# robin-karlsson0/pc-accumulation-lib

Measured on AMD Instinct MI355X. Metric: Mpoints/s projected+accumulated and BEV frames/s @256x256; 1/2/4/8 GPU, higher is better.
Workload: dtype f64; 1 GPU; KITTI-360 single forward cam, 120k pts/frame, 200 m horizon (~201 live frames, 5169634 stored pts), one 256x256x21 BEV per integrated frame; points_per_frame=120000, bev_px=256, view_m=80

## Files before the change

### include/pca.h

```cpp
#ifndef PCA_H
#define PCA_H

#include <stdint.h>

#ifdef __cplusplus
extern "C" {
#endif

#define PCA_VERSION 2

typedef struct pca_ctx pca_ctx;

typedef struct {
    double *x, *y, *z;
    float *intensity;
    uint32_t *rgbs;
    int32_t *inst;
    uint8_t *dyn;
    int64_t capacity;
    uint32_t *frame_box;
} pca_store;

#define PCA_STATUS_STORE_OVERFLOW 1u
#define PCA_STATUS_UV_OUT_OF_IMAGE 2u
#define PCA_STATUS_NEGATIVE_INTENSITY 4u
#define PCA_STATUS_LOOKBACK_TIMEOUT 8u
#define PCA_STATUS_LANES_BISECT_CAP 16u

int pca_version(void);
int pca_ctx_create(int device, pca_ctx **out);
void pca_ctx_destroy(pca_ctx *ctx);
const char *pca_last_error(pca_ctx *ctx);
int pca_status(pca_ctx *ctx, void *stream, uint32_t *status_out);
int pca_status_peek(pca_ctx *ctx, uint32_t *status_out);
const uint32_t *pca_status_mirror(pca_ctx *ctx);

typedef struct {
    const float *pts;
    const uint8_t *rgb;
    const uint8_t *sem;
    const uint8_t *sem_gt;
    int32_t n;
    int32_t reserved;
} pca_kitti_frame;

int pca_kitti_project_sample_filter(pca_ctx *ctx, const pca_kitti_frame *frames, int n_frames, const double P[12],
                                    int H, int W, const uint64_t filter_mask[4], const pca_store *store,
                                    int64_t *frame_off , int first_slot, void *stream);

#define PCA_SAMPLE_NEAREST 0
#define PCA_SAMPLE_BILINEAR 1
int pca_kitti_project_sample_filter_ex(pca_ctx *ctx, const pca_kitti_frame *frames, int n_frames, const double P[12],
                                       int H, int W, const uint64_t filter_mask[4], const pca_store *store,
                                       int64_t *frame_off , int first_slot, int sample_mode, void *stream);

int pca_nusc_sample_filter_transform(pca_ctx *ctx, const double *pc, const int64_t *cam_idx, int32_t n,
                                     const uint8_t *imgs, const uint8_t *sems, int ncam, int H, int W,
                                     const double T[16], const uint64_t filter_mask[4], const pca_store *store,
                                     int64_t *frame_off , int slot, void *stream);
int pca_nusc_sample_filter_transform_ex(pca_ctx *ctx, const double *pc, const int64_t *cam_idx, int32_t n,
                                        const uint8_t *imgs, const uint8_t *sems, int ncam, int H, int W,
                                        const double T[16], const uint64_t filter_mask[4], const pca_store *store,
                                        int64_t *frame_off , int slot, int sample_mode, void *stream);

typedef struct {
    const double *pc;
    const int64_t *cam_idx;
    const uint8_t *imgs;
    const uint8_t *sems;
    int32_t n;
    int32_t reserved;
    const double *T;
} pca_nusc_frame;
int pca_nusc_sample_filter_transform_batch(pca_ctx *ctx, const pca_nusc_frame *frames, int n_frames, int ncam, int H, int W,
                                           const uint64_t filter_mask[4], const pca_store *store, int64_t *frame_off ,
                                           int first_slot, int sample_mode, void *stream);

int pca_sample_bilinear(pca_ctx *ctx, const double *map , int H, int W, const double *uv , int32_t n,
                        double *out , void *stream);

int pca_nusc_project_cams(pca_ctx *ctx, const double *pc_lidar, int32_t n, const double T_ego_from_lidar[16],
                          const double T_glob_from_ego[16], const double *T_cam_from_glob, const double *K,
                          const double *wh, int ncam, double *pc_in_ego, double *uv, int64_t *cam_idx,
                          void *stream);

#define PCA_NUSC_MAX_SWEEPS 32
#define PCA_NUSC_MAX_SWEEP_BOXES 4096
#define PCA_NUSC_MAX_SWEEP_TILES 16384
typedef struct {
    int32_t row0, n_rows;
    int32_t box0, n_boxes;
    float lag, sweep;
    double T[12];
} pca_nusc_sweep;
typedef struct {
    double inv[12];
    double size[3];
    int32_t cls;
    int32_t track_key;
} pca_nusc_sweep_box;
int64_t pca_nusc_merge_sweeps_workspace_bytes(int64_t n_points, int n_boxes);
int pca_nusc_merge_sweeps(pca_ctx *ctx, const float *raw , int64_t n_points, const pca_nusc_sweep *sweeps,
                          int n_sweeps, const pca_nusc_sweep_box *boxes, int n_boxes, float center_radius,
                          double inside_limit, void *workspace , int64_t workspace_bytes,
                          float *points_out , int32_t *tally_out , void *stream);

int pca_retransform(pca_ctx *ctx, const pca_store *store, const int64_t *frame_off , int slot_begin,
                    int slot_end, const double *Ts, int n_T, void *stream);

int pca_retransform_batch_tail(pca_ctx *ctx, const pca_store *store, const int64_t *frame_off , int first_slot,
                               int n_frames, const double *Ts, void *stream);

int pca_mark_dynamic(pca_ctx *ctx, const pca_store *store, const int64_t *frame_off , const int32_t *slots,
                     const int32_t *inst_idx, int n_pairs, void *stream);

int64_t pca_voxel_dedup_workspace_bytes(int64_t max_points, int n_slots);
int pca_voxel_dedup(pca_ctx *ctx, const pca_store *store, int64_t *frame_off , int slot_begin, int slot_end,
                    double voxel_size, int64_t max_points, void *workspace , int64_t workspace_bytes,
                    void *stream);

int64_t pca_icp_workspace_bytes(int32_t max_points);
int pca_icp_register(pca_ctx *ctx, const float *src_pts , int32_t n_src, const float *tgt_pts ,
                     int32_t n_tgt, double max_corr_dist, const double init[16], int max_iter, double rel_fitness,
                     double rel_rmse, void *workspace , int64_t workspace_bytes, double T_out[16],
                     double *fitness, double *rmse, int *iterations, void *stream);

typedef struct {
    double origin[3];
    double R[9];
    double dx, dy;
    double view;
    double height_filter;
    double int_scaler, int_sep_scaler, int_mid_threshold;
    double rgb_fill;
    int32_t px;
    int32_t road_class;
    uint64_t dynobj_mask[4];
    int32_t intensity_div255;
    int32_t pad;
} pca_bev_params;

int64_t pca_bev_workspace_bytes(int64_t max_points, int px);

int pca_bev_generate(pca_ctx *ctx, const pca_store *store, const double *intensity64,
                     const int64_t *frame_off , int slot_begin, int slot_split, int slot_end,
                     int64_t max_points, const pca_bev_params *prm, const double *pending_T, int pending_slot_end,
                     void *workspace , int64_t workspace_bytes, double *planes ,
                     uint16_t *planes_f16 , void *stream);

#define PCA_BEV_EXTRA_PLANES 3
int pca_bev_generate_ex(pca_ctx *ctx, const pca_store *store, const double *intensity64,
                        const int64_t *frame_off , int slot_begin, int slot_split, int slot_end,
                        int64_t max_points, const pca_bev_params *prm, const double *pending_T, int pending_slot_end,
                        void *workspace , int64_t workspace_bytes, double *planes ,
                        uint16_t *planes_f16 , double *extra_planes , void *stream);

#define PCA_BEV_MAX_CHAIN 4
int pca_bev_generate_chain(pca_ctx *ctx, const pca_store *store, const double *intensity64,
                           const int64_t *frame_off , int slot_begin, int slot_split, int slot_end,
                           int64_t max_points, const pca_bev_params *prm, const double *pending_Ts,
                           const int *pending_slot_ends, int n_pending, int write_back, void *workspace ,
                           int64_t workspace_bytes, double *planes , uint16_t *planes_f16 ,
                           double *extra_planes , void *stream);

typedef struct {
    int32_t slot_begin, slot_split, slot_end, reserved;
    pca_bev_params prm;
    double *planes;
    uint16_t *planes_f16;
} pca_bev_job;
int pca_bev_generate_many(pca_ctx *ctx, const pca_store *store, const double *intensity64 ,
                          const int64_t *frame_off , const pca_bev_job *jobs, int n_jobs, int64_t max_points,
                          void *workspace , int64_t workspace_bytes, void *stream);

#define PCA_BEV_MAX_CLASS_GROUPS 16
typedef struct { uint64_t mask[4]; } pca_class_group;
int64_t pca_bev_class_workspace_bytes(int64_t max_points, int px);
int pca_bev_class_planes(pca_ctx *ctx, const pca_store *store, const int64_t *frame_off ,
                         int slot_begin, int slot_split, int slot_end, int64_t max_points,
                         const pca_bev_params *prm,
                         const pca_class_group *groups, int n_groups,
                         const double *pending_Ts, const int *pending_slot_ends, int n_pending,
                         void *workspace , int64_t workspace_bytes,
                         double *prob      ,
                         uint16_t *prob_f16,
                         uint32_t *counts  ,
                         void *stream);

int64_t pca_bev_elev_workspace_bytes(int64_t max_points, int px);
int pca_bev_elev_partition(pca_ctx *ctx, const pca_store *store, const int64_t *frame_off ,
                           int slot_begin, int slot_end, int64_t max_points,
                           const pca_bev_params *prm, double elev_thresh, int include_dyn,
                           const double *pending_Ts, const int *pending_slot_ends, int n_pending,
                           void *workspace , int64_t workspace_bytes,
                           double *elev      ,
                           uint8_t *observed ,
                           uint8_t *flags    ,
                           int64_t *counts   ,
                           void *stream);

int pca_image_to_nchw_f32(pca_ctx *ctx, const uint8_t *rgb , int H, int W, const float mean[3], const float std[3],
                          float *out , void *stream);

int pca_bev_warp(pca_ctx *ctx, const uint16_t *planes_f16 , uint16_t *out_f16 , int n_planes, int px,
                 double a_1, double a_2, double b_1, double b_2, void *stream);

int pca_host_ego_to_grid(const double *full, int F, const double R[9], double dx, double dy, double view, int px,
                         double *rows, int32_t *start);

typedef struct {
    double origin[3];
    double R[9];
    double dx, dy, view;
    int32_t px, reserved;
} pca_lane_view;
int64_t pca_lanes_workspace_bytes(int64_t n_vertices, int n_samples, int64_t cap_rows);
int pca_lanes_transform(pca_ctx *ctx, double *xyz , int64_t P, const double T[16], void *stream);
int pca_lanes_to_grid(pca_ctx *ctx, const double *xyz , const int32_t *vertex_lane , const int32_t *start ,
                      int64_t P, int32_t L, const pca_lane_view *views , int S, int64_t cap_rows,
                      double *rows , int32_t *row_lane , int64_t *n_rows , void *ws,
                      void *stream);

typedef struct pca_host_track pca_host_track;
typedef struct {
    const void *pts;
    const void *rgb;
    const void *sem;
    const void *sem_gt;
    int32_t n;
    uint32_t host_mask;
} pca_kitti_obs;
int pca_kitti_integrate(pca_ctx *ctx, const pca_kitti_obs *obs, const double P[12], int H, int W,
                        const uint64_t filter_mask[4], const pca_store *store, int64_t *frame_off , int slot,
                        int sample_mode, pca_host_track *track, const double *T_new_prev, double horizon, int64_t *evicted,
                        double *path_length, void *stream);
void pca_host_camera_cone(const double P[12], int H, int W, double cone[15]);
int pca_host_view_hull(int F, const double *then , const float *box , const double *cone ,
                       const double now[12], const pca_bev_params *prm, int *first, int *last);
int pca_bev_bin_range(pca_ctx *ctx, int slot_first, int slot_last_plus1);
int pca_bev_view_hint(pca_ctx *ctx, int slot0, int F, const double *then, const float *box, const double *cone, const double now[12],
                      const pca_bev_params *prm);
void pca_f32_box_decode(const uint32_t *rows , int n, float *box );

int pca_debug_bev_level1(const pca_ctx *ctx, int out[4]);
int pca_debug_icp_layout(int32_t n_src, int32_t n_tgt, int64_t out[16]);

int pca_k1_defer(pca_ctx *ctx, int on);
int pca_k1_flush(pca_ctx *ctx);
int pca_kitti_generate_bev(pca_ctx *ctx, const pca_store *store, const int64_t *frame_off , int slot_begin,
                           int slot_split, int slot_end, int64_t max_points, const pca_bev_params *prm,
                           const double *pending_Ts, const int *pending_slot_ends, int n_pending, int write_back,
                           void *workspace , int64_t workspace_bytes, uint16_t *planes_f16 ,
                           void *host_planes , const pca_host_track *track, double *traj_rows,
                           int32_t *traj_start, int32_t *n_rows, void *stream);

typedef struct {
    const pca_kitti_obs *obs; const double *P; int32_t H, W; const uint64_t *filter_mask; const pca_store *store;
    int64_t *frame_off; int32_t slot, sample_mode; pca_host_track *track; const double *T_new_prev; double horizon;
    int64_t evicted; double path_length; void *stream;
} pca_kitti_integrate_args;
int pca_kitti_integrate_v(pca_ctx *ctx, pca_kitti_integrate_args *a);
typedef struct {
    const pca_store *store; const int64_t *frame_off; int32_t slot_begin, slot_split, slot_end, pad0; int64_t max_points;
    const pca_bev_params *prm; const double *pending_Ts; const int *pending_slot_ends; int32_t n_pending, write_back;
    void *workspace; int64_t workspace_bytes; uint16_t *planes_f16; void *host_planes; const pca_host_track *track;
    double *traj_rows; int32_t *traj_start; int32_t n_rows, pad1; void *stream;
    int32_t hint_slot0, hint_F; const double *hint_then; const float *hint_box; const double *hint_cone; const double *hint_now;
    int32_t hinted, pad2;
} pca_kitti_generate_bev_args;
int pca_kitti_generate_bev_v(pca_ctx *ctx, pca_kitti_generate_bev_args *a);

int pca_host_stage_h2d(int n, const void *const *src, void *const *pinned, void *const *dev, const int64_t *bytes,
                       void *stream);

int pca_host_d2h_async(pca_ctx *ctx, const void *dev, void *pinned, int64_t bytes, void *stream);
int pca_host_d2h_wait(pca_ctx *ctx, int ticket);

#define PCA_DEFLATE_CHUNK_MAX 32768
#define PCA_DEFLATE_MAX_CHUNKS (1 << 20)
#define PCA_DEFLATE_BOUND(n) ((9 * (int64_t)(n) + 7) / 8 + 16)
typedef struct { int64_t offset; int32_t length; int32_t reserved; } pca_deflate_chunk;
int64_t pca_deflate_workspace_bytes(int64_t n_chunks);
int pca_deflate_chunks(pca_ctx *ctx, const void *src , const pca_deflate_chunk *chunk_table , int64_t n_chunks,
                       void *out , uint32_t *out_sizes , uint32_t *out_crcs , void *workspace ,
                       void *stream);
int pca_deflate_chunks_dyn(pca_ctx *ctx, const void *src , const pca_deflate_chunk *chunk_table , int64_t n_chunks,
                           void *out , uint32_t *out_sizes , uint32_t *out_crcs , void *workspace ,
                           void *stream);
uint32_t pca_host_crc32_combine(uint32_t crc_a, uint32_t crc_b, int64_t len_b);
int64_t pca_host_gzip_assemble(int32_t n_pieces, const void *const *piece, const int64_t *piece_bytes, const int64_t *raw_bytes,
                               const uint32_t *crc, void *out, int64_t out_cap);

typedef struct pca_host_track pca_host_track;
int pca_host_gemv4_probe(void *cblas_dgemv64, int mode, const double *T , const double *x , int64_t n,
                         double *y );
int pca_host_gemv4_mode(int mode);
int pca_host_incr_probe(void *cblas_dgemv64, const double *d, int64_t n, int64_t r0, int64_t r1, double *out);
int pca_host_incr_blocks(int on);
int pca_host_track_create(pca_host_track **out, void *cblas_dgemv64);
void pca_host_track_destroy(pca_host_track *t);
int64_t pca_host_track_len(const pca_host_track *t);
int64_t pca_host_track_n_segments(const pca_host_track *t);
const double *pca_host_track_poses(const pca_host_track *t);
const double *pca_host_track_segments(const pca_host_track *t);
int pca_host_track_set(pca_host_track *t, const double *poses , int64_t n, const double *segs, int64_t nd);
int pca_host_track_transform(pca_host_track *t, const double T[16]);
int pca_host_track_append(pca_host_track *t, const double pose[3]);
int pca_host_track_push_segment(pca_host_track *t, double *path_length);
int pca_host_track_incr(pca_host_track *t, double *out);
int64_t pca_host_track_evict_beyond(pca_host_track *t, double horizon, double path_length);
int64_t pca_host_track_step(pca_host_track *t, const double T_new_prev[16], double horizon, double *path_length);
int64_t pca_host_track_trigger(pca_host_track *t, double bev_horizon, int64_t previous_idx, double min_step);

enum {
    PCA_K_KITTI = 0, PCA_K_NUSC, PCA_K_PROJECT_CAMS, PCA_K_RETRANSFORM, PCA_K_MARK_DYNAMIC,
    PCA_K_BEV_BIN, PCA_K_BEV_SCAN, PCA_K_BEV_SCATTER, PCA_K_BEV_CELLS, PCA_K_BEV_CELLS_HEAVY, PCA_K_DEDUP, PCA_K_BEV_UNIT, PCA_K_ICP,
    PCA_K_BEV_CLASS_BIN, PCA_K_BEV_CLASS_CELLS, PCA_K_BEV_ELEV_BIN, PCA_K_BEV_ELEV_CELLS, PCA_K_COUNT
};
int pca_profile_enable(pca_ctx *ctx, int on);
int pca_profile_read(pca_ctx *ctx, int kernel_id, double *total_ms, int64_t *launches);

#ifdef __cplusplus
}
#endif
#endif
```

### pc-accumulation-lib_amd/bev_generator/bev_generator.py

```python
import os
import time
from abc import ABC, abstractmethod

import ctypes

import numpy as np

from pca_amd import host_logic as hl

SETS = ('present', 'future', 'full')
PLANES = ('road', 'intensity', 'r', 'g', 'b', 'dynamic', 'elevation')


class DeviceWindow:

    def __init__(self, store, split, origin, first=0, last=None, future_is_present=False):
        self.store = store
        self.split = int(split)
        self.origin = np.asarray(origin, dtype=np.float64)
        self.first = int(first)
        self.last = store.n_frames if last is None else int(last)
        self.future_is_present = bool(future_is_present)

    def part(self, name):
        return WindowPart(self, name)


class WindowPart:

    def __init__(self, window, name):
        self.window = window
        self.name = name

    def to_numpy(self):
        w = self.window
        rows = w.store.frame_rows()
        lo, hi = {'present': (w.first, w.split), 'future': (w.split, w.last), 'full': (w.first, w.last)}[self.name]
        if w.future_is_present:
            lo, hi = w.first, w.last
        out = np.concatenate(rows[lo:hi]) if hi > lo else np.zeros((0, 10))
        out[:, :3] = out[:, :3] - w.origin
        return out


class BEVGenerator(ABC):

    def __init__(self,
                 view_size: int,
                 pixel_size: int,
                 max_trans_radius: float = 0.,
                 zoom_thresh: float = 0.,
                 do_warp: bool = False,
                 int_scaler: float = 1.,
                 int_sep_scaler: float = 1.,
                 int_mid_threshold: float = 0.5,
                 height_filter=None):
        self.view_size = view_size
        self.pixel_size = pixel_size
        self.max_trans_radius = max_trans_radius
        self.zoom_thresh = zoom_thresh
        self.do_warp = do_warp
        self.do_aug = bool(self.max_trans_radius > 0. or self.zoom_thresh > 0.)
        self.int_scaler = int_scaler
        self.int_sep_scaler = int_sep_scaler
        self.int_mid_threshold = int_mid_threshold
        self.sem_idx = 7
        self.height_filter = height_filter
        if self.height_filter is not None:
            print("NOTE: Removes points above ego-vehicle height!")
        self._tmp = {}
        self._frame = None
        self._device_only = False
        self._out16 = None
        self._defer = None
        self._lane_defer = None

    def __getstate__(self):
        d = dict(self.__dict__)
        d['_tmp'] = {}
        d['_defer'] = None
        d['_lane_defer'] = None
        return d

    class _RasterBatch:
        def __init__(self, gen):
            self.gen = gen

        def __enter__(self):
            self.gen._defer = []
            return self

        def __exit__(self, exc_type, exc, tb):
            jobs, self.gen._defer = self.gen._defer, None
            if self.gen._lane_defer is not None:
                lane_jobs, self.gen._lane_defer = self.gen._lane_defer, None
                if exc_type is not None:
                    return False
                lanes = lane_jobs[0][0]
                assert all(j[0] is lanes for j in lane_jobs)
                lanes.to_grid([j[1] for j in lane_jobs], asynchronous=True, into=[j[2] for j in lane_jobs])
            if exc_type is None and jobs:
                store = jobs[0][0]
                assert all(j[0] is store for j in jobs)
                outs = [j[2] for j in jobs]
                base = outs[0]._base if outs[0]._base is not None else outs[0]
                px = int(jobs[0][1][1].px)
                contiguous = all(o.data_ptr() == base.data_ptr() + k * 21 * px * px * 2 for k, o in enumerate(outs))
                if len(jobs) > 1 and contiguous and base.numel() >= len(jobs) * 21 * px * px:
                    store.bev_many([j[1] for j in jobs], base.view(-1)[:len(jobs) * 21 * px * px].view(len(jobs), 21, px, px))
                else:
                    for _, (split, prm, first, last), out in jobs:
                        store.bev(split, prm, first_frame=first, last_frame=last, out16=out)
            return False

    def raster_batch(self):
        return BEVGenerator._RasterBatch(self)

    def _raster_params(self, origin, rot_mat, dx, dy, aug_view_size, intensity_div255):
        key = ('prm', bool(intensity_div255), self.pixel_size, self.height_filter, self.int_scaler,
               self.int_sep_scaler, self.int_mid_threshold, getattr(self, 'rgb_fill', 0))
        prm = self._tmp.get(key)
        if prm is None:
            from pca_amd.device_store import make_bev_params
            sem_idxs = getattr(self, 'sem_idxs', None) or {}
            dyn_cls = [sem_idxs[k] for k in ('car', 'truck', 'bus', 'motorcycle') if k in sem_idxs]
            prm = self._tmp[key] = make_bev_params(np.zeros(3), np.eye(3), 0., 0., 1., self.pixel_size,
                                                   self.height_filter, self.int_scaler, self.int_sep_scaler,
                                                   self.int_mid_threshold, sem_idxs.get('road', -1), dyn_cls,
                                                   intensity_div255, getattr(self, 'rgb_fill', 0))
        head = self._tmp.get(id(prm))
        if head is None:
            head = self._tmp[id(prm)] = np.frombuffer((ctypes.c_double * 15).from_address(ctypes.addressof(prm)), dtype=np.float64)
        head[0:3] = origin
        head[3:12] = np.asarray(rot_mat, dtype=np.float64).reshape(9)
        head[12], head[13], head[14] = dx, dy, aug_view_size
        return prm

    def _tmp_store(self, key):
        from pca_amd.device_store import DeviceStore
        if key not in self._tmp:
            self._tmp[key] = DeviceStore(capacity=1 << 16, max_frames=4)
        return self._tmp[key]

    def rasterise(self, pc_present, pc_future, pc_full, rot_mat, dx, dy, aug_view_size, want_f64=False, out16=None):
        if isinstance(pc_present, WindowPart):
            w = pc_present.window
            prm = self._raster_params(w.origin, rot_mat, dx, dy, aug_view_size, w.store.intensity_div255)
            if self._defer is not None and out16 is not None and not want_f64 and not w.future_is_present:
                from pca_amd._lib import PcaBevParams
                self._defer.append((w.store, (w.split, PcaBevParams.from_buffer_copy(prm), w.first, w.last), out16))
                return out16, None
            return w.store.bev(w.split, prm, want_f64=want_f64, first_frame=w.first, last_frame=w.last, out16=out16)
        zero = np.zeros(3)
        prm = self._raster_params(zero, rot_mat, dx, dy, aug_view_size, False)
        st = self._tmp_store('pf')
        i64 = st.load_rows([pc_present, pc_future])
        a16, a64 = st.bev(1, prm, want_f64=want_f64, intensity64=i64)
        st2 = self._tmp_store('full')
        i64 = st2.load_rows([pc_full])
        b16, b64 = st2.bev(1, prm, want_f64=want_f64, intensity64=i64)
        a16[14:21] = b16[0:7]
        if want_f64:
            a64[14:21] = b64[0:7]
        return a16, a64

    @abstractmethod
    def generate_bev(self, pc_present, pc_future, pc_full, trajs_present, trajs_future, trajs_full,
                     gt_lane_trajs=None):
        pass

    def generate(self,
                 pcs: dict,
                 trajs: dict,
                 rot_ang: float = 0.,
                 trans_dx: float = 0.,
                 trans_dy: float = 0.,
                 zoom_scalar: float = 1.,
                 do_warping: bool = False,
                 device_only: bool = False,
                 out=None):
        pc_present, pc_future, pc_full = self.extract_pc_dict(pcs)
        ego_present, ego_future, ego_full = self.extract_ego_traj_dict(trajs)
        oth_present, oth_future, oth_full = self.extract_other_traj_dicts(trajs)
        lanes = self.extract_gt_lane_dicts(trajs) if 'gt_lanes' in trajs.keys() else None

        aug_view_size = zoom_scalar * self.view_size
        if do_warping is False:
            rot_ang = hl.heading_rot_ang(ego_present)
        rot_mat = hl.rotation_matrix_3d(rot_ang)

        def to_grid(traj_list):
            return [hl.transform_traj(t, rot_mat, trans_dx, trans_dy, aug_view_size, self.pixel_size, mutate=False)
                    for t in traj_list]

        split = trajs.get('_ego_split')
        if split is not None and pc_future is not None:
            ego_p, ego_f, ego_a = hl.transform_ego_split(ego_full, split, rot_mat, trans_dx, trans_dy, aug_view_size,
                                                        self.pixel_size)
            trajs_present = [ego_p] + to_grid(oth_present)
            trajs_future = [ego_f] + to_grid(oth_future)
            trajs_full = [ego_a] + to_grid(oth_full)
        else:
            trajs_present = to_grid([ego_present] + oth_present)
        if lanes is not None and not isinstance(lanes, list):
            from pca_amd.lanes import LaneView, PendingLanes
            view = LaneView(lanes.origin, rot_mat, trans_dx, trans_dy, aug_view_size, self.pixel_size)
            if self._defer is not None and device_only:
                if self._lane_defer is None:
                    self._lane_defer = []
                pending = PendingLanes()
                self._lane_defer.append((lanes.lanes, view, pending))
                lanes = pending
            else:
                lanes = lanes.lanes.to_grid([view], asynchronous=device_only)[0]
                if not device_only:
                    lanes = lanes.resolve()
        elif lanes is not None:
            lanes = [lane for lane in to_grid(lanes) if lane.shape[0] > 0]
        if pc_future is None:
            raise UnboundLocalError("local variable 'trajs_future' referenced before assignment")
        if split is None:
            trajs_future = to_grid([ego_future] + oth_future)
            trajs_full = to_grid([ego_full] + oth_full)

        self._frame = (rot_mat, trans_dx, trans_dy, aug_view_size)
        self._device_only = device_only
        self._out16 = out if device_only else None
        return self.generate_bev(pc_present, pc_future, pc_full, trajs_present, trajs_future, trajs_full, lanes)

    def preprocess_pc_and_trajs(self, pc, trajs, rot_ang, trans_dx, trans_dy, aug_view_size):
        rot_mat = hl.rotation_matrix_3d(rot_ang)
        pc = self.geometric_transform(pc, rot_ang, trans_dx, trans_dy, aug_view_size)
        out_trajs = [hl.transform_traj(t, rot_mat, trans_dx, trans_dy, aug_view_size, self.pixel_size)
                     for t in trajs]
        if self.height_filter is not None:
            pc = pc[pc[:, 2] < self.height_filter]
        return self.pos2grid(pc, aug_view_size), out_trajs

    def generate_rand_aug(self, pcs: dict, trajs: dict, do_warping: bool = True, device_only: bool = False, out=None,
                          worker: int = 0):
        np.random.seed(((os.getpid() + int(worker)) * int(time.time())) % 123456789)
        rot_ang = 2 * np.pi * np.random.random()
        trans_r = self.max_trans_radius * np.random.random()
        trans_ang = 2 * np.pi * np.random.random()
        trans_dx = trans_r * np.cos(trans_ang)
        trans_dy = trans_r * np.sin(trans_ang)
        zoom_scalar = np.random.normal(0, 0.1)
        zoom_scalar = 1 + min(max(zoom_scalar, -self.zoom_thresh), self.zoom_thresh)
        return self.generate(pcs, trajs, rot_ang, trans_dx, trans_dy, zoom_scalar, do_warping, device_only, out)

    def generate_multiproc(self, bev_gen_inputs, device_only: bool = False, out=None, worker: int = 0):
        pcs, trajs = bev_gen_inputs
        if self.do_aug:
            return self.generate_rand_aug(pcs, trajs, device_only=device_only, out=out, worker=worker)
        return self.generate(pcs, trajs, device_only=device_only, out=out)

    def generate_rand_aug_multiproc(self, bev_gen_inputs):
        pcs, trajs = bev_gen_inputs
        return self.generate_rand_aug(pcs, trajs, do_warping=True)

    def geometric_transform(self, pc_mat, rot_ang, trans_dx, trans_dy, aug_view_size, is_traj=False):
        rot_mat = self.rotation_matrix_3d(rot_ang)
        pc_mat[:, :3] = np.matmul(rot_mat, pc_mat[:, :3].T).T
        pc_mat[:, 0] += trans_dx
        pc_mat[:, 1] += trans_dy
        if is_traj:
            return self.crop_trajectory(pc_mat, aug_view_size)
        return self.crop_view(pc_mat, aug_view_size)

    @staticmethod
    def crop_view(pc_mat, aug_view_size):
        h = 0.5 * aug_view_size
        pc_mat = pc_mat[np.logical_and(pc_mat[:, 0] > -h, pc_mat[:, 0] < h)]
        return pc_mat[np.logical_and(pc_mat[:, 1] > -h, pc_mat[:, 1] < h)]

    def crop_trajectory(self, traj, aug_view_size, thresh=1e-4):
        return hl.crop_trajectory(traj, aug_view_size, thresh)

    @staticmethod
    def point_in_box(pnt_x, pnt_y, box_x0, box_y0, box_x1, box_y1):
        return (box_x0 < pnt_x and pnt_x < box_x1) and (box_y0 < pnt_y and pnt_y < box_y1)

    def cal_intersec_pnt(self, x0, y0, x1, y1, bbox, thresh=1e-4):
        return hl.bisect_box_crossing(x0, y0, x1, y1, bbox, thresh)

    @staticmethod
    def partition_semantic_pc(pc_mat, sems, sem_idx):
        mask = np.isin(pc_mat[:, sem_idx], list(sems))
        return pc_mat[mask], pc_mat[~mask]

    @staticmethod
    def dirichlet_dist_expectation(gridmaps, obs_weight=1):
        g = np.stack(gridmaps) * obs_weight + 1.
        g /= np.sum(g, axis=0)
        return [g[k] for k in range(g.shape[0])]

    @staticmethod
    def warp_dense_probmaps(probmaps, a_1, a_2, b_1, b_2):
        return hl.warp_dense_probmaps(probmaps, a_1, a_2, b_1, b_2)

    def warp_sparse_points(self, pnts, a_1, a_2, b_1, b_2, i_mid, j_mid, i_warp, j_warp):
        return hl.warp_sparse_points(pnts, a_1, a_2, j_warp, j_mid, self.pixel_size)

    @staticmethod
    def warp_point(x, y, a_1, a_2, b_1, b_2, I, J):
        return hl.warp_point(x, y, a_1, a_2, b_1, b_2, I, J)

    def warp_points(self, pnt_list, a_1, a_2, b_1, b_2, I, J):
        return [hl.warp_point(p[0], p[1], a_1, a_2, b_1, b_2, I, J) for p in pnt_list]

    @staticmethod
    def get_random_warp_params(mean_ratio, max_ratio, I, J):
        return hl.get_random_warp_params(mean_ratio, max_ratio, I, J)

    @staticmethod
    def cal_warp_params(idx_0, idx_1, idx_max):
        return hl.cal_warp_params(idx_0, idx_1, idx_max)

    def warp_trajs(self, trajs, a_1, a_2, b_1, b_2, i_mid, j_mid, i_warp, j_warp):
        return [self.warp_sparse_points(t, a_1, a_2, b_1, b_2, i_mid, j_mid, i_warp, j_warp) for t in trajs]

    @staticmethod
    def extract_pc_dict(pcs: dict):
        return pcs['pc_present'], pcs['pc_future'], pcs['pc_full']

    @staticmethod
    def extract_ego_traj_dict(trajs: dict) -> tuple:
        return trajs['ego_traj_present'], trajs['ego_traj_future'], trajs['ego_traj_full']

    @staticmethod
    def extract_other_traj_dicts(trajs: dict) -> tuple:
        return trajs['other_trajs_present'], trajs['other_trajs_future'], trajs['other_trajs_full']

    @staticmethod
    def extract_gt_lane_dicts(trajs: dict) -> tuple:
        return trajs['gt_lanes']

    @staticmethod
    def extract_aug_dict(augs: dict):
        return augs['max_translation_radius'], augs['zoom_threshold']

    @staticmethod
    def rotation_matrix_3d(ang):
        return hl.rotation_matrix_3d(ang)

    def pos2grid(self, pc_mat, view_size):
        return hl.pos2grid_inplace(pc_mat, view_size, self.pixel_size)

    @abstractmethod
    def viz_bev(self):
        pass
```

### pc-accumulation-lib_amd/csrc/pca_api.hip

```cpp
#include <stdio.h>
#include <cmath>
#include "pca_common.h"

__global__ __launch_bounds__(256) void pca_fetch_block_kernel(const uint4 *src, uint4 *dst, int64_t n16)
{
    for (int64_t i = (int64_t)blockIdx.x * 256 + threadIdx.x; i < n16; i += (int64_t)gridDim.x * 256) dst[i] = src[i];
}

int pca_fetch_block(pca_ctx *ctx, const void *mapped_host, int64_t offset, void *dev, int64_t bytes, hipStream_t s)
{
    if (bytes <= 0) return 0;
    void *src = nullptr;
    PCA_CHECK(ctx, hipHostGetDevicePointer(&src, const_cast<void *>(mapped_host), 0));
    src = reinterpret_cast<char *>(src) + offset;
    const int64_t n16 = (bytes + 15) / 16;
    const int grid = (int)((n16 + 255) / 256 < 64 ? (n16 + 255) / 256 : 64);
    hipLaunchKernelGGL(pca_fetch_block_kernel, dim3(grid), dim3(256), 0, s, reinterpret_cast<const uint4 *>(src),
                       reinterpret_cast<uint4 *>(dev), n16);
    PCA_CHECK(ctx, hipGetLastError());
    return 0;
}

int pca_dev_grow(pca_ctx *ctx, void **p, int64_t *cap, int64_t need, hipStream_t s)
{
    if (need <= *cap) return 0;
    PCA_CHECK(ctx, hipStreamSynchronize(s));
    if (*p) PCA_CHECK(ctx, hipFree(*p));
    *p = nullptr; *cap = 0;
    const int64_t want = need + need / 4;
    PCA_CHECK(ctx, hipMalloc(p, (size_t)want));
    *cap = want;
    return 0;
}

int pca_ctx_reserve_tiles(pca_ctx *ctx, int64_t tiles, hipStream_t s)
{
    if (tiles <= ctx->tile_cap) return 0;
    PCA_CHECK(ctx, hipStreamSynchronize(s));
    if (ctx->tile_state) PCA_CHECK(ctx, hipFree(ctx->tile_state));
    ctx->tile_cap = tiles * 2 > 4096 ? tiles * 2 : 4096;
    PCA_CHECK(ctx, hipMalloc(&ctx->tile_state, sizeof(uint64_t) * ctx->tile_cap));
    PCA_CHECK(ctx, hipMemsetAsync(ctx->tile_state, 0, sizeof(uint64_t) * ctx->tile_cap, s));
    ctx->epoch = 0;
    return 0;
}

uint32_t pca_ctx_next_epoch(pca_ctx *ctx, hipStream_t s)
{
    ctx->epoch = (ctx->epoch + 1) & 0x3fffffu;
    if (ctx->epoch == 0) {
        (void)hipMemsetAsync(ctx->tile_state, 0, sizeof(uint64_t) * ctx->tile_cap, s);
        ctx->epoch = 1;
    }
    return ctx->epoch;
}

void pca_prof_begin(pca_ctx *ctx, int kid, hipStream_t s)
{
    pca_ctx::Ev e;
    if (!ctx->free_evs.empty()) { e = ctx->free_evs.back(); ctx->free_evs.pop_back(); }
    else { (void)hipEventCreate(&e.a); (void)hipEventCreate(&e.b); }
    e.kid = kid;
    (void)hipEventRecord(e.a, s);
    ctx->evs.push_back(e);
}

void pca_prof_end(pca_ctx *ctx, hipStream_t s) { (void)hipEventRecord(ctx->evs.back().b, s); }

static void prof_fold(pca_ctx *ctx)
{
    for (auto &e : ctx->evs) {
        (void)hipEventSynchronize(e.b);
        float ms = 0.f;
        if (hipEventElapsedTime(&ms, e.a, e.b) == hipSuccess) { ctx->prof_ms[e.kid] += ms; ctx->prof_n[e.kid]++; }
        ctx->free_evs.push_back(e);
    }
    ctx->evs.clear();
}

extern "C" {

void pca_host_camera_cone(const double P[12], int H, int W, double cone[15])
{
    const double a00 = P[0], a01 = P[1], a02 = P[2], a10 = P[4], a11 = P[5], a12 = P[6], a20 = P[8], a21 = P[9], a22 = P[10];
    const double c00 = a11 * a22 - a12 * a21, c01 = a02 * a21 - a01 * a22, c02 = a01 * a12 - a02 * a11;
    const double c10 = a12 * a20 - a10 * a22, c11 = a00 * a22 - a02 * a20, c12 = a02 * a10 - a00 * a12;
    const double c20 = a10 * a21 - a11 * a20, c21 = a01 * a20 - a00 * a21, c22 = a00 * a11 - a01 * a10;
    const double id = 1.0 / (a00 * c00 + a01 * c10 + a02 * c20);
    const double inv[9] = {c00 * id, c01 * id, c02 * id, c10 * id, c11 * id, c12 * id, c20 * id, c21 * id, c22 * id};
    for (int r = 0; r < 3; ++r) cone[r] = -(inv[3 * r] * P[3] + inv[3 * r + 1] * P[7] + inv[3 * r + 2] * P[11]);
    const double us[2] = {-1.5, (double)W + 0.5}, vs[2] = {-1.5, (double)H + 0.5};
    for (int k = 0; k < 4; ++k) {
        const double u = us[k & 1], v = vs[k >> 1];
        for (int r = 0; r < 3; ++r) cone[3 + 3 * k + r] = inv[3 * r] * u + inv[3 * r + 1] * v + inv[3 * r + 2];
    }
}

void pca_f32_box_decode(const uint32_t *rows, int n, float *box)
{
    for (int f = 0; f < n; ++f)
        for (int k = 0; k < 3; ++k) {
            const uint32_t l = rows[6 * f + 2 * k], h = rows[6 * f + 2 * k + 1];
            const bool have = h != 0u;
            box[6 * f + 2 * k] = have ? pca_f32_from_ordered(~l) : 1.0f;
            box[6 * f + 2 * k + 1] = have ? pca_f32_from_ordered(h) : -1.0f;
        }
}

int pca_host_view_hull(int F, const double *then, const float *box, const double *cone, const double now[12],
                       const pca_bev_params *prm, int *first, int *last)
{
    if (F < 0 || !then || !now || !prm || !first || !last) return -1;
    const double h = 0.5 * prm->view + 0.01;
    auto visible = [&](int f) -> bool {
        const double *m = then + 12 * (size_t)f;
        const double a00 = m[0], a01 = m[1], a02 = m[2], a10 = m[4], a11 = m[5], a12 = m[6], a20 = m[8], a21 = m[9], a22 = m[10];
        const double c00 = a11 * a22 - a12 * a21, c01 = a02 * a21 - a01 * a22, c02 = a01 * a12 - a02 * a11;
        const double c10 = a12 * a20 - a10 * a22, c11 = a00 * a22 - a02 * a20, c12 = a02 * a10 - a00 * a12;
        const double c20 = a10 * a21 - a11 * a20, c21 = a01 * a20 - a00 * a21, c22 = a00 * a11 - a01 * a10;
        const double id = 1.0 / (a00 * c00 + a01 * c10 + a02 * c20);
        const double inv[9] = {c00 * id, c01 * id, c02 * id, c10 * id, c11 * id, c12 * id, c20 * id, c21 * id, c22 * id};
        double Q[6], q[2];
        {
            double Mr[6], Mt[2];
            for (int r = 0; r < 2; ++r) {
                for (int c = 0; c < 3; ++c) Mr[3 * r + c] = now[4 * r] * inv[c] + now[4 * r + 1] * inv[3 + c] + now[4 * r + 2] * inv[6 + c];
                Mt[r] = now[4 * r + 3] - (Mr[3 * r] * m[3] + Mr[3 * r + 1] * m[7] + Mr[3 * r + 2] * m[11]);
            }
            const double tx = Mt[0] - prm->origin[0], ty = Mt[1] - prm->origin[1];
            q[0] = prm->R[0] * tx + prm->R[1] * ty + prm->dx;
            q[1] = prm->R[3] * tx + prm->R[4] * ty + prm->dy;
            for (int c = 0; c < 3; ++c) {
                Q[c] = prm->R[0] * Mr[c] + prm->R[1] * Mr[3 + c];
                Q[3 + c] = prm->R[3] * Mr[c] + prm->R[4] * Mr[3 + c];
            }
        }
        for (int k = 0; k < 6; ++k) if (!std::isfinite(Q[k])) return true;
        if (!std::isfinite(q[0]) || !std::isfinite(q[1])) return true;
        for (int axis = 0; axis < 2; ++axis)
            for (int side = 0; side < 2; ++side) {
                const double s = side ? -1.0 : 1.0;
                const double *row = Q + 3 * axis;
                if (cone) {
                    const double ua = s * (row[0] * cone[0] + row[1] * cone[1] + row[2] * cone[2] + q[axis]);
                    bool out = ua >= h;
                    for (int k = 0; k < 4 && out; ++k) {
                        const double *d = cone + 3 + 3 * k;
                        out = s * (row[0] * d[0] + row[1] * d[1] + row[2] * d[2]) >= 0.0;
                    }
                    if (out) return false;
                }
                if (box) {
                    const float *b = box + 6 * (size_t)f;
                    if (b[0] <= b[1] && b[2] <= b[3] && b[4] <= b[5]) {
                        double lo = s * q[axis];
                        for (int c = 0; c < 3; ++c) {
                            const double x0 = s * row[c] * (double)b[2 * c], x1 = s * row[c] * (double)b[2 * c + 1];
                            lo += x0 < x1 ? x0 : x1;
                        }
                        if (lo >= h) return false;
                    }
                }
            }
        return true;
    };
    int a = 0, b = F - 1;
    while (a <= b && !visible(a)) ++a;
    while (b >= a && !visible(b)) --b;
    if (a > b) { *first = -1; *last = -1; } else { *first = a; *last = b; }
    return 0;
}

int pca_bev_view_hint(pca_ctx *ctx, int slot0, int F, const double *then, const float *box, const double *cone, const double now[12],
                      const pca_bev_params *prm)
{
    if (!ctx) return -1;
    int first = 0, last = 0;
    if (pca_host_view_hull(F, then, box, cone, now, prm, &first, &last)) return -1;
    if (first == 0 && last == F - 1) return 0;
    if (first < 0) { first = 0; last = -1; }
    ctx->bin_first = slot0 + first; ctx->bin_end = slot0 + last + 1; ctx->bin_valid = true;
    return 1;
}

int pca_bev_bin_range(pca_ctx *ctx, int slot_first, int slot_last_plus1)
{
    if (!ctx) return -1;
    ctx->bin_first = slot_first; ctx->bin_end = slot_last_plus1; ctx->bin_valid = slot_last_plus1 >= slot_first;
    return 0;
}

static inline bool box_inside(double x, double y, double lo, double hi) { return lo < x && x < hi && lo < y && y < hi; }

int pca_host_ego_to_grid(const double *full, int F, const double R[9], double dx, double dy, double view, int px,
                         double *rows, int32_t *start)
{
    if (F < 2) { if (F == 1 && start) start[0] = 0; return 0; }
    const double h = 0.5 * view, lo = -h, pxd = (double)px, half_px = 0.5 * pxd;
    auto rot = [&](const double *p, double &x, double &y, double &z) {
        x = fma(R[2], p[2], fma(R[1], p[1], R[0] * p[0] + 0.0)) + dx;
        y = fma(R[5], p[2], fma(R[4], p[1], R[3] * p[0] + 0.0)) + dy;
        z = fma(R[8], p[2], fma(R[7], p[1], R[6] * p[0] + 0.0));
    };
    auto emit = [&](int m, double x, double y, double z) {
        rows[3 * m + 0] = floor(x / view * pxd + half_px);
        rows[3 * m + 1] = floor(y / view * pxd + half_px);
        rows[3 * m + 2] = z;
    };
    int m = 0;
    double ax, ay, az, bx, by, bz;
    rot(full, ax, ay, az);
    bool a_in = box_inside(ax, ay, lo, h);
    for (int k = 0; k + 1 < F; ++k) {
        rot(full + 3 * (k + 1), bx, by, bz);
        const bool b_in = box_inside(bx, by, lo, h);
        start[k] = m;
        if (a_in) emit(m++, ax, ay, az);
        if (a_in != b_in) {
            double x0 = ax, y0 = ay, x1 = bx, y1 = by, xm = 0.0, ym = 0.0, gap = __builtin_huge_val();
            while (gap > 1e-4) {
                xm = 0.5 * (x0 + x1);
                ym = 0.5 * (y0 + y1);
                const bool p0_in = box_inside(x0, y0, lo, h), mid_in = box_inside(xm, ym, lo, h);
                if (mid_in == p0_in) { gap = sqrt((xm - x0) * (xm - x0) + (ym - y0) * (ym - y0)); x0 = xm; y0 = ym; }
                else { gap = sqrt((xm - x1) * (xm - x1) + (ym - y1) * (ym - y1)); x1 = xm; y1 = ym; }
            }
            emit(m++, xm, ym, az);
        }
        ax = bx; ay = by; az = bz; a_in = b_in;
    }
    start[F - 1] = m;
    return m;
}

int pca_profile_enable(pca_ctx *ctx, int on)
{
    if (!ctx) return -1;
    prof_fold(ctx);
    ctx->profiling = on < 0 ? 0 : (on > 2 ? 2 : on);
    if (on) for (int k = 0; k < PCA_K_COUNT; ++k) { ctx->prof_ms[k] = 0; ctx->prof_n[k] = 0; }
    return 0;
}

int pca_profile_read(pca_ctx *ctx, int kernel_id, double *total_ms, int64_t *launches)
{
    if (!ctx || kernel_id < 0 || kernel_id >= PCA_K_COUNT) return -1;
    prof_fold(ctx);
    if (total_ms) *total_ms = ctx->prof_ms[kernel_id];
    if (launches) *launches = ctx->prof_n[kernel_id];
    return 0;
}

int pca_version(void) { return PCA_VERSION; }

int pca_ctx_create(int device, pca_ctx **out)
{
    if (!out) return -1;
    *out = nullptr;
    pca_ctx *ctx = new pca_ctx();
    ctx->device = device;
#define PCA_CREATE_STEP(expr)                                                                                          \
    do {                                                                                                               \
        const hipError_t e_ = (expr);                                                                                  \
        if (e_ != hipSuccess) {                                                                                        \
            fprintf(stderr, "pca_ctx_create(device %d): %s failed: %s\n", device, #expr, hipGetErrorString(e_));       \
            delete ctx;                                                                                                \
            return -1;                                                                                                 \
        }                                                                                                              \
    } while (0)
    PCA_CREATE_STEP(hipSetDevice(device));
    PCA_CREATE_STEP(hipMalloc(&ctx->ticket, sizeof(PcaStatusBlock)));
    PCA_CREATE_STEP(hipMemset(ctx->ticket, 0, sizeof(PcaStatusBlock)));
    PCA_CREATE_STEP(hipHostMalloc(&ctx->status_host, sizeof(uint32_t)));
    PCA_CREATE_STEP(hipHostMalloc(&ctx->status_mirror, PCA_STATUS_BITS * sizeof(uint32_t), hipHostMallocMapped));
    PCA_CREATE_STEP(hipHostMalloc(&ctx->heavy_hint, 4 * sizeof(uint32_t), hipHostMallocMapped));
    int n_cu = 0;
    if (hipDeviceGetAttribute(&n_cu, hipDeviceAttributeMultiprocessorCount, device) == hipSuccess && n_cu > 0) ctx->n_cu = n_cu;
    *ctx->heavy_hint = 1;
    ctx->heavy_hint[1] = ctx->heavy_hint[2] = ctx->heavy_hint[3] = 0;
    for (int b = 0; b < PCA_STATUS_BITS; ++b) ctx->status_mirror[b] = 0;
    PCA_CREATE_STEP(hipHostGetDevicePointer(reinterpret_cast<void **>(&ctx->heavy_hint_dev), ctx->heavy_hint, 0));
    PCA_CREATE_STEP(hipHostGetDevicePointer(reinterpret_cast<void **>(&ctx->status_mirror_dev), ctx->status_mirror, 0));
    PCA_CREATE_STEP(hipMemcpy(reinterpret_cast<char *>(ctx->ticket) + offsetof(PcaStatusBlock, mirror), &ctx->status_mirror_dev, sizeof(void *), hipMemcpyHostToDevice));
#undef PCA_CREATE_STEP
    *out = ctx;
    return 0;
}

void pca_ctx_destroy(pca_ctx *ctx)
{
    if (!ctx) return;
    (void)hipSetDevice(ctx->device);
    if (ctx->tile_state) (void)hipFree(ctx->tile_state);
    if (ctx->ticket) (void)hipFree(ctx->ticket);
    if (ctx->k1_ws) (void)hipFree(ctx->k1_ws);
    for (int i = 0; i < 2; ++i) {
        if (ctx->k1_pin[i]) (void)hipHostFree(ctx->k1_pin[i]);
        if (ctx->k1_pin_ev[i]) (void)hipEventDestroy(ctx->k1_pin_ev[i]);
    }
    if (ctx->k1_frames_dev) (void)hipFree(ctx->k1_frames_dev);
    if (ctx->k1_tiny) (void)hipFree(ctx->k1_tiny);
    for (auto &st : ctx->stage) {
        if (st.done) { (void)hipEventSynchronize(st.done); (void)hipEventDestroy(st.done); }
        if (st.pin) (void)hipHostFree(st.pin);
        if (st.dev) (void)hipFree(st.dev);
    }
    if (ctx->bevm_pin) (void)hipHostFree(ctx->bevm_pin);
    if (ctx->bevm_ev) (void)hipEventDestroy(ctx->bevm_ev);
    for (auto &e : ctx->d2h_done) if (e) (void)hipEventDestroy(e);
    if (ctx->d2h_go) (void)hipEventDestroy(ctx->d2h_go);
    if (ctx->d2h_stream) (void)hipStreamDestroy(ctx->d2h_stream);
    if (ctx->h2d_done[0]) (void)hipEventDestroy(ctx->h2d_done[0]);
    if (ctx->h2d_stream[0]) { (void)hipStreamSynchronize(ctx->h2d_stream[0]); (void)hipStreamDestroy(ctx->h2d_stream[0]); }
    if (ctx->k1n_ws) (void)hipFree(ctx->k1n_ws);
    if (ctx->k1n_desc_dev) (void)hipFree(ctx->k1n_desc_dev);
    if (ctx->k1n_pin) (void)hipHostFree(ctx->k1n_pin);
    if (ctx->k1n_ev) (void)hipEventDestroy(ctx->k1n_ev);
    if (ctx->icp_cnt) (void)hipFree(ctx->icp_cnt);
    if (ctx->icp_host) (void)hipHostFree(ctx->icp_host);
    if (ctx->status_host) (void)hipHostFree(ctx->status_host);
    if (ctx->status_mirror) (void)hipHostFree(ctx->status_mirror);
    if (ctx->heavy_hint) (void)hipHostFree(ctx->heavy_hint);
    prof_fold(ctx);
    for (auto &e : ctx->free_evs) { (void)hipEventDestroy(e.a); (void)hipEventDestroy(e.b); }
    delete ctx;
}

const char *pca_last_error(pca_ctx *ctx) { return ctx ? ctx->err.c_str() : "null context"; }

int pca_status(pca_ctx *ctx, void *stream, uint32_t *status_out)
{
    if (!ctx || !status_out) return -1;
    if (pca_k1_flush_pending(ctx)) return -1;
    hipStream_t s = (hipStream_t)stream;
    PCA_CHECK(ctx, hipSetDevice(ctx->device));
    PCA_CHECK(ctx, hipMemcpyAsync(ctx->status_host, ctx->ticket + 1, sizeof(uint32_t), hipMemcpyDeviceToHost, s));
    PCA_CHECK(ctx, hipMemsetAsync(ctx->ticket + 1, 0, sizeof(uint32_t), s));
    PCA_CHECK(ctx, hipStreamSynchronize(s));
    *status_out = *ctx->status_host;
    for (int b = 0; b < PCA_STATUS_BITS; ++b) {
        if (__atomic_load_n(&ctx->status_mirror[b], __ATOMIC_RELAXED)) *status_out |= 1u << b;
        __atomic_store_n(&ctx->status_mirror[b], 0u, __ATOMIC_RELAXED);
    }
    return 0;
}

int pca_status_peek(pca_ctx *ctx, uint32_t *status_out)
{
    if (!ctx || !status_out) return -1;
    uint32_t st = 0;
    for (int b = 0; b < PCA_STATUS_BITS; ++b)
        if (__atomic_load_n(&ctx->status_mirror[b], __ATOMIC_RELAXED)) st |= 1u << b;
    *status_out = st;
    return 0;
}

const uint32_t *pca_status_mirror(pca_ctx *ctx) { return ctx ? ctx->status_mirror : nullptr; }

}
```

### pc-accumulation-lib_amd/csrc/pca_session.hip

```cpp
#include <vector>

#include "pca_common.h"

int pca_stage_copy(const void *const *src, void *const *dst, const int64_t *bytes, int n);

extern "C" {

int pca_kitti_integrate(pca_ctx *ctx, const pca_kitti_obs *obs, const double P[12], int H, int W,
                        const uint64_t filter_mask[4], const pca_store *store, int64_t *frame_off, int slot, int sample_mode,
                        pca_host_track *track, const double *T_new_prev, double horizon, int64_t *evicted,
                        double *path_length, void *stream)
{
    if (!ctx) return -1;
    if (!obs || obs->n < 0 || !P || !filter_mask || !store || !frame_off) { ctx->err = "kitti_integrate: bad arguments"; return -1; }
    if (track && (!T_new_prev || !evicted || !path_length)) { ctx->err = "kitti_integrate: the pose track needs T_new_prev and its outputs"; return -1; }
    hipStream_t s = (hipStream_t)stream;
    PCA_CHECK(ctx, hipSetDevice(ctx->device));
    if (pca_k1_flush_pending(ctx)) return -1;
    const void *in[4] = {obs->pts, obs->rgb, obs->sem, obs->sem_gt};
    const int64_t size[4] = {16ll * obs->n, 3ll * H * W, 1ll * H * W, 1ll * obs->n};
    const void *dev[4] = {in[0], in[1], in[2], in[3]};
    int64_t off[4] = {0, 0, 0, 0}, total = 0;
    for (int k = 0; k < 4; ++k) {
        if (!(in[k] && ((obs->host_mask >> k) & 1u))) continue;
        if (size[k] > 0) { off[k] = total; total += pca_align256(size[k]); }
        else dev[k] = nullptr;
    }
    pca_ctx::Stage *slot_st = nullptr;
    if (total > 0) {
        pca_ctx::Stage &st = ctx->stage[ctx->stage_next++ % PCA_STAGE_DEPTH];
        if (st.busy) { PCA_CHECK(ctx, hipEventSynchronize(st.done)); st.busy = false; }
        if (st.cap < total) {
            if (st.pin) PCA_CHECK(ctx, hipHostFree(st.pin));
            if (st.dev) PCA_CHECK(ctx, hipFree(st.dev));
            st.pin = st.dev = nullptr; st.cap = 0;
            const int64_t cap = total + total / 4;
            PCA_CHECK(ctx, hipHostMalloc(&st.pin, (size_t)cap));
            PCA_CHECK(ctx, hipMalloc(&st.dev, (size_t)cap));
            st.cap = cap;
        }
        if (!st.done) PCA_CHECK(ctx, hipEventCreateWithFlags(&st.done, hipEventDisableTiming));
        const void *src[4]; void *dst[4]; int64_t bytes[4]; int m = 0;
        for (int k = 0; k < 4; ++k)
            if (in[k] && ((obs->host_mask >> k) & 1u) && size[k] > 0) {
                src[m] = in[k]; dst[m] = (char *)st.pin + off[k]; bytes[m] = size[k]; ++m;
                dev[k] = (char *)st.dev + off[k];
            }
        pca_stage_copy(src, dst, bytes, m);
        const int64_t side_min = PCA_ENV_ONCE("PCA_H2D_SIDE_MIN", 256ll << 10);
        if (total >= side_min) {
            if (!ctx->h2d_stream[0]) PCA_CHECK(ctx, hipStreamCreateWithFlags(&ctx->h2d_stream[0], hipStreamNonBlocking));
            if (!ctx->h2d_done[0]) PCA_CHECK(ctx, hipEventCreateWithFlags(&ctx->h2d_done[0], hipEventDisableTiming));
            PCA_CHECK(ctx, hipMemcpyAsync(st.dev, st.pin, (size_t)total, hipMemcpyHostToDevice, ctx->h2d_stream[0]));
            PCA_CHECK(ctx, hipEventRecord(ctx->h2d_done[0], ctx->h2d_stream[0]));
            PCA_CHECK(ctx, hipStreamWaitEvent(s, ctx->h2d_done[0], 0));
        } else {
            PCA_CHECK(ctx, hipMemcpyAsync(st.dev, st.pin, (size_t)total, hipMemcpyHostToDevice, s));
        }
        slot_st = &st;
    }
    pca_kitti_frame fr;
    fr.pts = (const float *)dev[0]; fr.rgb = (const uint8_t *)dev[1]; fr.sem = (const uint8_t *)dev[2];
    fr.sem_gt = (const uint8_t *)dev[3]; fr.n = obs->n; fr.reserved = 0;
    const bool plain = obs->n > 0 && sample_mode == PCA_SAMPLE_NEAREST && (fr.sem_gt || ((int64_t)H * W * 3 >= 4 && fr.rgb && fr.sem)) &&
                       obs->n <= (1 << 20);
    if (ctx->k1_defer && plain) {
        pca_ctx::K1Pending &pd = ctx->k1_pend;
        pd.fr = fr;
        for (int i = 0; i < 12; ++i) pd.P[i] = P[i];
        pd.H = H; pd.W = W;
        for (int i = 0; i < 4; ++i) pd.filt[i] = filter_mask[i];
        pd.store = *store; pd.frame_off = frame_off; pd.slot = slot; pd.sample_mode = sample_mode; pd.stream = s;
        pd.stage_idx = slot_st ? (int)(slot_st - ctx->stage) : -1;
        pd.valid = true;
    } else {
        const int rc = pca_kitti_project_sample_filter_ex(ctx, &fr, 1, P, H, W, filter_mask, store, frame_off, slot, sample_mode, stream);
        if (slot_st) {
            const hipError_t e = hipEventRecord(slot_st->done, s);
            if (e == hipSuccess) slot_st->busy = true;
            else {
                (void)hipStreamSynchronize(s);
                if (rc == 0) { ctx->err = std::string("kitti_integrate: hipEventRecord(stage done): ") + hipGetErrorString(e); return -1; }
            }
        }
        if (rc != 0) return rc;
    }
    if (track) *evicted = pca_host_track_step(track, T_new_prev, horizon, path_length);
    return 0;
}

int pca_kitti_generate_bev(pca_ctx *ctx, const pca_store *store, const int64_t *frame_off, int slot_begin, int slot_split,
                           int slot_end, int64_t max_points, const pca_bev_params *prm, const double *pending_Ts,
                           const int *pending_slot_ends, int n_pending, int write_back, void *workspace,
                           int64_t workspace_bytes, uint16_t *planes_f16, void *host_planes, const pca_host_track *track,
                           double *traj_rows, int32_t *traj_start, int32_t *n_rows, void *stream)
{
    if (!ctx) return -1;
    if (!prm || !planes_f16 || !track || !traj_rows || !traj_start || !n_rows) { ctx->err = "kitti_generate_bev: bad arguments"; return -1; }
    const int64_t F = pca_host_track_len(track);
    if (F != slot_end - slot_begin) { ctx->err = "kitti_generate_bev: the pose track and the window disagree about the number of frames"; return -1; }
    static thread_local std::vector<double> rel;
    rel.resize((size_t)(3 * (F > 0 ? F : 1)));
    const double *Hp = pca_host_track_poses(track);
    for (int64_t f = 0; f < F; ++f)
        for (int k = 0; k < 3; ++k) rel[(size_t)(3 * f + k)] = Hp[4 * f + k] - prm->origin[k];
    *n_rows = pca_host_ego_to_grid(rel.data(), (int)F, prm->R, prm->dx, prm->dy, prm->view, prm->px, traj_rows, traj_start);
    if (pca_bev_generate_chain(ctx, store, nullptr, frame_off, slot_begin, slot_split, slot_end, max_points, prm, pending_Ts,
                               pending_slot_ends, n_pending, write_back, workspace, workspace_bytes, nullptr, planes_f16,
                               nullptr, stream) != 0)
        return -1;
    if (!host_planes) return 0;
    return pca_host_d2h_async(ctx, planes_f16, host_planes, 21ll * prm->px * prm->px * 2, stream);
}

int pca_kitti_integrate_v(pca_ctx *ctx, pca_kitti_integrate_args *a)
{
    if (!ctx) return -1;
    if (!a) { ctx->err = "kitti_integrate_v: no argument block"; return -1; }
    return pca_kitti_integrate(ctx, a->obs, a->P, a->H, a->W, a->filter_mask, a->store, a->frame_off, a->slot, a->sample_mode,
                               a->track, a->T_new_prev, a->horizon, &a->evicted, &a->path_length, a->stream);
}

int pca_kitti_generate_bev_v(pca_ctx *ctx, pca_kitti_generate_bev_args *a)
{
    if (!ctx) return -1;
    if (!a) { ctx->err = "kitti_generate_bev_v: no argument block"; return -1; }
    a->hinted = 0;
    if (a->hint_F > 0 && !(a->n_pending > 0 && a->write_back)) {
        const int rc = pca_bev_view_hint(ctx, a->hint_slot0, a->hint_F, a->hint_then, a->hint_box, a->hint_cone, a->hint_now, a->prm);
        if (rc < 0) { ctx->err = "kitti_generate_bev_v: bad view hint"; return -1; }
        a->hinted = rc;
    }
    return pca_kitti_generate_bev(ctx, a->store, a->frame_off, a->slot_begin, a->slot_split, a->slot_end, a->max_points, a->prm,
                                  a->pending_Ts, a->pending_slot_ends, a->n_pending, a->write_back, a->workspace,
                                  a->workspace_bytes, a->planes_f16, a->host_planes, a->track, a->traj_rows, a->traj_start,
                                  &a->n_rows, a->stream);
}

}
```

### pc-accumulation-lib_amd/kitti360_sem_pc_accum.py

```python
import os

import numpy as np

from sem_pc_accum import SemanticPointCloudAccumulator

_MODS = None


def _mods():
    global _MODS
    if _MODS is None:
        import ctypes

        import torch
        from bev_generator.sem_bev import LazyBev, SemBEVGenerator, _PendingCopy
        from pca_amd import host_logic
        from pca_amd._lib import PcaKittiObs
        _MODS = (ctypes, torch, LazyBev, _PendingCopy, SemBEVGenerator, host_logic, PcaKittiObs)
    return _MODS


class Kitti360SemanticPointCloudAccumulator(SemanticPointCloudAccumulator):

    def __init__(self, horizon_dist: float, calib_params: dict, icp_threshold: float, semseg_onnx_path: str,
                 semseg_filters: list, sem_idxs: dict, use_gt_sem: bool, bev_params: dict):
        super().__init__(horizon_dist, icp_threshold, semseg_onnx_path, semseg_filters, sem_idxs, use_gt_sem,
                         bev_params)
        self.H_velo_cam = calib_params['h_velo_cam']
        self.P_cam_frame = calib_params['p_cam_frame']
        self.P_velo_frame = calib_params['p_velo_frame']
        self._gpu_icp = None
        self._uploader = None
        self._cobs = None
        self._ga = None
        self._ga_traj = None
        self._fast = os.environ.get('PCA_FAST_CALLS', '1') != '0'
        self._defer_k1 = self._fast and os.environ.get('PCA_FUSE_K1', '1') != '0'
        self._prev_sweep = None
        self._sweep_dev = None
        self.pose_provider = self._default_pose_provider()

    def _default_pose_provider(self):
        import os
        path = os.environ.get('PCA_KITTI_T_FILE')
        if path:
            Ts = iter(np.load(path))
            return lambda pc: next(Ts)
        spec = os.environ.get('PCA_POSE_PROVIDER')
        if spec == 'gpu_icp':
            return self._gpu_icp_pose
        if spec == 'open3d':
            return self._icp_pose
        if spec:
            import importlib
            mod, _, fn = spec.partition(':')
            return getattr(importlib.import_module(mod), fn)
        return self._icp_pose

    def _gpu_icp_pose(self, pc):
        import torch
        from pca_amd.icp import GpuIcp
        if self._gpu_icp is None:
            self._gpu_icp = GpuIcp()
        if not isinstance(pc, torch.Tensor) and getattr(pc, 'dtype', None) == np.float32 and pc.ndim == 2 and pc.shape[1] == 4:
            new = self._upload([('icp_pts', pc)])[0]
            self._sweep_dev = (pc, new)
        else:
            new = GpuIcp.to_device(pc)
        if self._prev_sweep is None:
            self._prev_sweep = new
        reg = self._gpu_icp.register(self._prev_sweep, new, self.icp_threshold, self.icp_trans_init)
        self._prev_sweep = new
        return reg.transformation

    def _icp_pose(self, pc):
        try:
            import open3d as o3d
        except ImportError as e:
            raise ImportError('the KITTI-360 flow takes its poses from Open3D ICP, as the reference does, and open3d is '
                              'not importable; name another pose source: accumulator.pose_provider = callable, '
                              'PCA_KITTI_T_FILE=<poses.npy>, PCA_POSE_PROVIDER=<module>:<callable> or '
                              'PCA_POSE_PROVIDER=gpu_icp (device ICP, not bit-compatible with Open3D)') from e
        pcd_new = self.pc2pcd(pc)
        if self.pcd_prev is None:
            self.pcd_prev = pcd_new
        reg = o3d.pipelines.registration.registration_icp(
            self.pcd_prev, pcd_new, self.icp_threshold, self.icp_trans_init,
            o3d.pipelines.registration.TransformationEstimationPointToPlane())
        self.pcd_prev = pcd_new
        return reg.transformation

    def _frame_tensors(self, rgb, pc, sem_gt):
        import torch
        dev = self.store.device
        dtype_np = {torch.float32: np.float32, torch.uint8: np.uint8}
        want, host = {}, []

        def up(name, a, dtype):
            a = getattr(a, 'dev', a)
            if isinstance(a, torch.Tensor):
                if a.device != dev or a.dtype != dtype or not a.is_contiguous():
                    a = a.to(device=dev, dtype=dtype).contiguous()
                want[name] = a
            else:
                want[name] = len(host)
                host.append((name, np.ascontiguousarray(a, dtype=dtype_np[dtype])))

        up('pts', pc, torch.float32)
        semseg = None
        if sem_gt is None:
            img = rgb if isinstance(rgb, torch.Tensor) or hasattr(rgb, 'dev') else np.asarray(rgb)
            up('rgb', img, torch.uint8)
            if getattr(self.semseg_model, 'accepts_device', False):
                if not isinstance(want['rgb'], torch.Tensor):
                    want['rgb'] = self._upload(host[want['rgb']:want['rgb'] + 1])[0]
                    host.pop()
                semseg = self.semseg_model.pred(want['rgb'])[0, 0]
            else:
                semseg = self.semseg_model.pred(rgb)[0, 0]
            up('sem', semseg, torch.uint8)
        else:
            sg = sem_gt if isinstance(sem_gt, torch.Tensor) else np.asarray(sem_gt)[:, -1]
            up('sem_gt', sg, torch.uint8)
        if host:
            for (name, _), t in zip(host, self._upload(host)):
                want[name] = t
        frame = want
        H, W = tuple(frame['sem'].shape) if sem_gt is None else (1, 1)
        return frame, semseg, H, W

    def _upload(self, items):
        if self._uploader is None:
            from pca_amd.ingest import PinnedUploader
            self._uploader = PinnedUploader(self.store.device)
        return self._uploader.upload_many(items)

    def _obs_pointers(self, rgb, pc, sem_gt):
        _, torch, _, _, _, _, PcaKittiObs = _mods()
        dev = self.store.device
        obs = self._cobs
        if obs is None:
            obs = self._cobs = PcaKittiObs()
        keep, mask = [], 0

        def put(a, np_dtype, t_dtype, bit):
            nonlocal mask
            if not isinstance(a, torch.Tensor):
                own = getattr(a, '__dict__', {})
                d = own.get('dev') if isinstance(own.get('dev'), torch.Tensor) else own.get('_dev')
                if isinstance(d, torch.Tensor):
                    a = d
                elif '_host' in own and '_dev' in own:
                    a = a.host
            if isinstance(a, torch.Tensor):
                if a.device != dev or a.dtype != t_dtype or not a.is_contiguous():
                    a = a.to(device=dev, dtype=t_dtype).contiguous()
                keep.append(a)
                return a.data_ptr(), tuple(a.shape)
            a = np.ascontiguousarray(a, dtype=np_dtype)
            keep.append(a)
            mask |= bit
            return a.ctypes.data, a.shape

        obs.pts, shape = put(pc, np.float32, torch.float32, 1)
        if len(shape) != 2 or shape[1] != 4:
            raise ValueError('pc must be (N, 4): x, y, z, intensity')
        obs.n = int(shape[0])
        semseg = None
        if sem_gt is None:
            if getattr(self.semseg_model, 'accepts_device', False) and not isinstance(rgb, torch.Tensor) \
                    and getattr(rgb, '__dict__', {}).get('_dev') is None:
                return None
            obs.rgb, ishape = put(rgb, np.uint8, torch.uint8, 2)
            src = keep[-1] if getattr(self.semseg_model, 'accepts_device', False) else rgb
            semseg = self.semseg_model.pred(src)[0, 0]
            obs.sem, sshape = put(semseg, np.uint8, torch.uint8, 4)
            if len(ishape) != 3 or ishape[2] != 3 or tuple(ishape[:2]) != tuple(sshape):
                raise ValueError(f'image {tuple(ishape)} and class map {tuple(sshape)} do not fit together')
            obs.sem_gt = None
            H, W = int(sshape[0]), int(sshape[1])
        else:
            sg = sem_gt if isinstance(sem_gt, torch.Tensor) else np.asarray(sem_gt)[:, -1]
            obs.sem_gt, gshape = put(sg, np.uint8, torch.uint8, 8)
            if tuple(gshape) != (obs.n, ):
                raise ValueError('sem_gt must hold one label per point')
            obs.rgb = obs.sem = None
            H, W = 1, 1
        obs.host_mask = mask
        return obs, semseg, H, W, keep

    def integrate(self, observations: list):
        rgb, pc, sem_gt = observations[0]
        if not self.use_gt_sem:
            sem_gt = None
        T_new_prev = np.asarray(self.pose_provider(pc), dtype=np.float64)
        self.T_prev_origin = np.matmul(self.T_prev_origin, T_new_prev)
        if self._sweep_dev is not None:
            host, dev = self._sweep_dev
            self._sweep_dev = None
            if host is pc:
                pc = dev
        fast = self._obs_pointers(rgb, pc, sem_gt) if self._fast else None
        general = self._frame_tensors(rgb, pc, sem_gt) if fast is None else None
        if len(self._track) > 0:
            self.update_sem_pcs(T_new_prev)
        if fast is not None:
            obs, semseg, H, W, keep = fast
            if self._defer_k1 != getattr(self.store.ctx, 'k1_defer', False):
                self.store.set_defer_k1(self._defer_k1)
            idx, path_length = self.store.append_kitti_obs(obs, self.P_velo_frame, H, W, self.semseg_filters, self.sample_mode,
                                                           self._track, T_new_prev, self.horizon_dist, keep=keep)
            del keep
            if idx is None:
                idx, path_length = self._track.step(T_new_prev, self.horizon_dist)
        else:
            frame, semseg, H, W = general
            self.store.append_kitti([frame], self.P_velo_frame, H, W, self.semseg_filters, sample_mode=self.sample_mode)
            idx, path_length = self._track.step(T_new_prev, self.horizon_dist)
        self.rgbs.append(rgb)
        self.semsegs.append(semseg)
        if idx:
            self.store.evict(idx)
            self.rgbs = self.rgbs[idx:]
            self.semsegs = self.semsegs[idx:]
        if path_length is not None:
            print(f'    #pc {self.store.n_frames} |', f'path length {path_length:.2f}')
        self._after_integrate()
        return idx

    def integrate_many(self, batch: list, max_frames_per_launch: int = 64):
        if self.voxel_dedup:
            return [self.integrate(obs) for obs in batch]
        out = []
        for b0 in range(0, len(batch), max_frames_per_launch):
            out += self._integrate_batch(batch[b0:b0 + max_frames_per_launch])
        return out

    def _integrate_batch(self, batch):
        from pca_amd.ingest import check_ring_lifetime
        check_ring_lifetime([item for observations in batch for item in observations[0]], len(batch))
        frames, Ts, shape = [], [], None
        for observations in batch:
            rgb, pc, sem_gt = observations[0]
            if not self.use_gt_sem:
                sem_gt = None
            T_new_prev = np.asarray(self.pose_provider(pc), dtype=np.float64)
            self.T_prev_origin = np.matmul(self.T_prev_origin, T_new_prev)
            if self._sweep_dev is not None:
                host, dev = self._sweep_dev
                self._sweep_dev = None
                if host is pc:
                    pc = dev
            frame, semseg, H, W = self._frame_tensors(rgb, pc, sem_gt)
            if shape not in (None, (H, W)):
                raise ValueError('integrate_many: all images of a batch must have one size')
            shape = (H, W)
            frames.append(frame)
            Ts.append(T_new_prev)
            self.rgbs.append(rgb)
            self.semsegs.append(semseg)
        self.store.flush_pending()
        self.store.append_kitti(frames, self.P_velo_frame, shape[0], shape[1], self.semseg_filters,
                                sample_mode=self.sample_mode)
        self.store.retransform_batch(np.stack(Ts), len(frames))
        removed, total = [], 0
        for T_new_prev in Ts:
            idx, path_length = self._track.step(T_new_prev, self.horizon_dist)
            if path_length is not None:
                print(f'    #pc {len(self._track)} |', f'path length {path_length:.2f}')
            removed.append(idx)
            total += idx
            self._integrated += 1
        self.store.poll_status()
        if total:
            self.store.evict(total)
            self.rgbs = self.rgbs[total:]
            self.semsegs = self.semsegs[total:]
        return removed

    def obs2sem_vec_space(self, rgb, pc, sem_gt=None) -> tuple:
        from pca_amd.device_store import DeviceStore
        T_new_prev = np.asarray(self.pose_provider(pc), dtype=np.float64)
        self.T_prev_origin = np.matmul(self.T_prev_origin, T_new_prev)
        main, self._store = self._store, DeviceStore(capacity=max(len(pc), 1), max_frames=2)
        try:
            frame, semseg, H, W = self._frame_tensors(rgb, pc, sem_gt)
            self._store.append_kitti([frame], self.P_velo_frame, H, W, self.semseg_filters)
            rows = self._store.rows(0)
        finally:
            self._store = main
        return rows, [0., 0., 0.], semseg, T_new_prev

    def generate_bev(self, present_idx: int = None, bev_num: int = 1, gen_future: bool = False):
        if bev_num == 1 and gen_future and self._fast_bev_ok(present_idx):
            return [self._generate_bev_fast(present_idx)]
        pcs, trajs = self._window_inputs(present_idx, gen_future)
        return self._run_bev(pcs, trajs, bev_num)

    def generate_bev_device(self, present_idx: int, out=None):
        if self._fast_bev_ok(present_idx):
            return self._generate_bev_fast(present_idx, out=out, to_host=False)
        pcs, trajs = self._window_inputs(present_idx, True)
        return self.sem_bev_generator.generate(pcs, trajs, device_only=True, out=out)

    def _fast_bev_ok(self, present_idx):
        gen = self.sem_bev_generator
        if not self._fast or type(gen) is not _mods()[4] or gen.do_aug or gen.do_warp or self._store is None \
                or getattr(self._track, '_h', None) is None or os.environ.get('PCA_SYNC_BEV') or getattr(gen, 'sem_planes', None):
            return False
        if not isinstance(present_idx, (int, np.integer)):
            return False
        n = self._store.n_frames
        split = int(present_idx) if present_idx >= 0 else n + int(present_idx)
        return 0 < split < n and n == len(self._track)

    def _generate_bev_fast(self, present_idx, out=None, to_host=True):
        C, torch, LazyBev, _PendingCopy, _, hl, _ = _mods()
        st, gen, track = self.store, self.sem_bev_generator, self._track
        ctx = st.ctx
        st.poll_status()
        n = st.n_frames
        present_idx = int(present_idx)
        split = present_idx if present_idx >= 0 else n + present_idx
        lo = max(split - 2, 0)
        near = track.poses_window(lo, split + 1)
        origin = near[split - lo]
        rot_mat = hl.rotation_matrix_3d(hl.heading_rot_ang(near[:split - lo] - origin))
        px = gen.pixel_size
        prm = gen._raster_params(origin, rot_mat, 0., 0., 1. * gen.view_size, st.intensity_div255)
        max_points = st.bev_workspace(px)
        n_pend, pend_T, pend_ends, write_back = st.bev_pending(0, n)
        if out is None:
            out = torch.empty((21, px, px), dtype=torch.float16, device=st.device)
        else:
            assert out.dtype == torch.float16 and out.is_contiguous() and tuple(out.shape) == (21, px, px)
        host = torch.empty((1, 21, px, px), dtype=torch.float16, pin_memory=True) if to_host else None
        tb = self._ga_traj
        if tb is None or tb[0].shape[0] < 2 * n or tb[1].shape[0] < n + 1:
            tb = self._ga_traj = (np.empty((4 * n + 64, 3)), np.zeros(2 * n + 64, dtype=np.int32))
            self._ga_traj_addr = (tb[0].ctypes.data, tb[1].ctypes.data)
        start = tb[1]
        cst = st.c_store()
        a = self._ga
        if a is None:
            from pca_amd._lib import PcaKittiGenerateBevArgs
            a = self._ga = PcaKittiGenerateBevArgs()
            self._ga_const = None
        pend_T, pend_ends = st._pend_T, st._pend_ends
        const = (id(cst), id(st.frame_off), id(prm), id(pend_T), id(pend_ends), id(st._ws), track._h)
        if const != self._ga_const:
            a.store, a.frame_off, a.prm = C.addressof(cst), st.frame_off.data_ptr(), C.addressof(prm)
            a.pending_Ts, a.pending_slot_ends = C.addressof(pend_T), C.addressof(pend_ends)
            a.workspace, a.workspace_bytes = st._ws.data_ptr(), st._ws.numel()
            a.track = getattr(track._h, 'value', track._h)
            self._ga_const = const
            self._ga_keep = (cst, st.frame_off, prm, pend_T, pend_ends, st._ws)
        a.slot_begin, a.slot_split, a.slot_end, a.max_points = st.head, st.head + split, st.head + n, max_points
        a.n_pending, a.write_back = n_pend, write_back
        a.planes_f16, a.host_planes = out.data_ptr(), (None if host is None else host.data_ptr())
        a.traj_rows, a.traj_start = self._ga_traj_addr
        a.stream = ctx.stream_int() or None
        a.hint_F = st.view_hint_into(a, 0, n)
        ticket = ctx.lib.pca_kitti_generate_bev_v(ctx.h, C.addressof(a))
        if ticket < 0:
            ctx.check(ticket)
        st.hints_taken += a.hinted
        st.bev_done(write_back)
        rows = tb[0][:a.n_rows].copy()
        empty = np.zeros((0, 3))
        ego_p = rows[:start[split - 1]].copy() if split >= 2 else empty
        ego_f = rows[start[split]:].copy() if n - split >= 2 else empty
        if not to_host:
            return {'planes_f16': out, 'trajs_present': [ego_p], 'trajs_future': [ego_f], 'trajs_full': [rows]}
        return LazyBev(host, 0, _PendingCopy(ctx, ticket, (out, host)), ([ego_p], [ego_f], [rows]))
```

### pc-accumulation-lib_amd/pca_amd/_lib.py

```python
import ctypes as C
import os
import threading

import numpy as np

_HERE = os.path.dirname(os.path.abspath(__file__))
LIB_PATH = os.path.join(_HERE, 'libpca_hip.so')

STATUS_STORE_OVERFLOW = 1
STATUS_UV_OUT_OF_IMAGE = 2
STATUS_NEGATIVE_INTENSITY = 4
STATUS_LOOKBACK_TIMEOUT = 8
STATUS_LANES_BISECT_CAP = 16
SAMPLE_MODES = {'nearest': 0, 'bilinear': 1}

EXPORTS = ('pca_version', 'pca_ctx_create', 'pca_ctx_destroy', 'pca_last_error', 'pca_status', 'pca_status_peek', 'pca_status_mirror',
           'pca_kitti_project_sample_filter', 'pca_kitti_project_sample_filter_ex',
           'pca_nusc_sample_filter_transform', 'pca_nusc_sample_filter_transform_ex', 'pca_nusc_sample_filter_transform_batch', 'pca_sample_bilinear', 'pca_nusc_project_cams',
           'pca_nusc_merge_sweeps_workspace_bytes', 'pca_nusc_merge_sweeps', 'pca_retransform', 'pca_retransform_batch_tail',
           'pca_mark_dynamic',
           'pca_bev_workspace_bytes', 'pca_bev_generate', 'pca_bev_generate_ex', 'pca_bev_generate_chain', 'pca_bev_generate_many', 'pca_bev_class_workspace_bytes', 'pca_bev_class_planes', 'pca_bev_elev_workspace_bytes', 'pca_bev_elev_partition', 'pca_bev_warp', 'pca_lanes_workspace_bytes', 'pca_lanes_transform', 'pca_lanes_to_grid', 'pca_image_to_nchw_f32', 'pca_voxel_dedup_workspace_bytes', 'pca_voxel_dedup', 'pca_icp_workspace_bytes', 'pca_icp_register', 'pca_host_ego_to_grid',
           'pca_host_gemv4_probe', 'pca_host_gemv4_mode', 'pca_host_incr_probe', 'pca_host_incr_blocks', 'pca_host_track_create', 'pca_host_track_destroy', 'pca_host_track_len', 'pca_host_track_n_segments',
           'pca_host_track_poses', 'pca_host_track_segments', 'pca_host_track_set', 'pca_host_track_transform',
           'pca_host_track_append', 'pca_host_track_push_segment', 'pca_host_track_incr', 'pca_host_track_evict_beyond',
           'pca_host_track_step', 'pca_host_track_trigger', 'pca_host_stage_h2d', 'pca_host_d2h_async', 'pca_host_d2h_wait',
           'pca_deflate_workspace_bytes', 'pca_deflate_chunks', 'pca_deflate_chunks_dyn', 'pca_host_crc32_combine', 'pca_host_gzip_assemble',
           'pca_kitti_integrate', 'pca_kitti_generate_bev', 'pca_k1_defer', 'pca_k1_flush', 'pca_host_camera_cone', 'pca_host_view_hull', 'pca_bev_bin_range', 'pca_bev_view_hint', 'pca_kitti_integrate_v', 'pca_kitti_generate_bev_v', 'pca_f32_box_decode', 'pca_debug_bev_level1', 'pca_debug_icp_layout',
           'pca_profile_enable', 'pca_profile_read')

KERNEL_IDS = ('kitti_project_sample_filter', 'nusc_sample_filter_transform', 'nusc_project_cams', 'retransform',
              'mark_dynamic', 'bev_bin', 'bev_scan', 'bev_scatter', 'bev_cells', 'bev_cells_heavy', 'voxel_dedup', 'bev_unit', 'icp', 'bev_class_bin', 'bev_class_cells', 'bev_elev_bin', 'bev_elev_cells')
BEV_EXTRA_PLANES = ('elevation_max', 'elevation_mean', 'intensity_mean')


class PcaStore(C.Structure):
    _fields_ = [('x', C.c_void_p), ('y', C.c_void_p), ('z', C.c_void_p), ('intensity', C.c_void_p),
                ('rgbs', C.c_void_p), ('inst', C.c_void_p), ('dyn', C.c_void_p), ('capacity', C.c_int64),
                ('frame_box', C.c_void_p)]


class PcaKittiIntegrateArgs(C.Structure):
    _fields_ = [('obs', C.c_void_p), ('P', C.c_void_p), ('H', C.c_int32), ('W', C.c_int32), ('filter_mask', C.c_void_p),
                ('store', C.c_void_p), ('frame_off', C.c_void_p), ('slot', C.c_int32), ('sample_mode', C.c_int32),
                ('track', C.c_void_p), ('T_new_prev', C.c_void_p), ('horizon', C.c_double), ('evicted', C.c_int64),
                ('path_length', C.c_double), ('stream', C.c_void_p)]


class PcaKittiGenerateBevArgs(C.Structure):
    _fields_ = [('store', C.c_void_p), ('frame_off', C.c_void_p), ('slot_begin', C.c_int32), ('slot_split', C.c_int32),
                ('slot_end', C.c_int32), ('pad0', C.c_int32), ('max_points', C.c_int64), ('prm', C.c_void_p),
                ('pending_Ts', C.c_void_p), ('pending_slot_ends', C.c_void_p), ('n_pending', C.c_int32), ('write_back', C.c_int32),
                ('workspace', C.c_void_p), ('workspace_bytes', C.c_int64), ('planes_f16', C.c_void_p), ('host_planes', C.c_void_p),
                ('track', C.c_void_p), ('traj_rows', C.c_void_p), ('traj_start', C.c_void_p), ('n_rows', C.c_int32),
                ('pad1', C.c_int32), ('stream', C.c_void_p), ('hint_slot0', C.c_int32), ('hint_F', C.c_int32),
                ('hint_then', C.c_void_p), ('hint_box', C.c_void_p), ('hint_cone', C.c_void_p), ('hint_now', C.c_void_p),
                ('hinted', C.c_int32), ('pad2', C.c_int32)]


class PcaKittiObs(C.Structure):
    _fields_ = [('pts', C.c_void_p), ('rgb', C.c_void_p), ('sem', C.c_void_p), ('sem_gt', C.c_void_p),
                ('n', C.c_int32), ('host_mask', C.c_uint32)]


class PcaKittiFrame(C.Structure):
    _fields_ = [('pts', C.c_void_p), ('rgb', C.c_void_p), ('sem', C.c_void_p), ('sem_gt', C.c_void_p),
                ('n', C.c_int32), ('reserved', C.c_int32)]


class PcaNuscFrame(C.Structure):
    _fields_ = [('pc', C.c_void_p), ('cam_idx', C.c_void_p), ('imgs', C.c_void_p), ('sems', C.c_void_p),
                ('n', C.c_int32), ('reserved', C.c_int32), ('T', C.POINTER(C.c_double))]


class PcaBevParams(C.Structure):
    _fields_ = [('origin', C.c_double * 3), ('R', C.c_double * 9), ('dx', C.c_double), ('dy', C.c_double),
                ('view', C.c_double), ('height_filter', C.c_double), ('int_scaler', C.c_double),
                ('int_sep_scaler', C.c_double), ('int_mid_threshold', C.c_double), ('rgb_fill', C.c_double),
                ('px', C.c_int32), ('road_class', C.c_int32), ('dynobj_mask', C.c_uint64 * 4),
                ('intensity_div255', C.c_int32), ('pad', C.c_int32)]


class PcaClassGroup(C.Structure):
    _fields_ = [('mask', C.c_uint64 * 4)]


BEV_MAX_CLASS_GROUPS = 16


class PcaBevJob(C.Structure):
    _fields_ = [('slot_begin', C.c_int32), ('slot_split', C.c_int32), ('slot_end', C.c_int32), ('reserved', C.c_int32),
                ('prm', PcaBevParams), ('planes', C.c_void_p), ('planes_f16', C.c_void_p)]


def class_mask(classes):
    m = [0, 0, 0, 0]
    for c in classes or []:
        c = int(c)
        if 0 <= c < 256:
            m[c >> 6] |= 1 << (c & 63)
    return (C.c_uint64 * 4)(*m)


def f64_array(a, n):
    a = np.ascontiguousarray(a, dtype=np.float64).ravel()
    assert a.size == n, (a.size, n)
    return (C.c_double * n)(*a.tolist())


_lib = None


def load():
    global _lib
    if _lib is not None:
        return _lib
    if not os.path.exists(LIB_PATH):
        raise RuntimeError(f'{LIB_PATH} not found: build it with `python -c "import __graft_entry__ as g; '
                           f'g.build()"` or `make -C pc-accumulation-lib_amd/csrc` (no CPU fallback exists)')
    import torch
    lib = C.CDLL(LIB_PATH)
    vp, i32, i64 = C.c_void_p, C.c_int, C.c_int64
    lib.pca_version.restype = C.c_int
    lib.pca_ctx_create.argtypes = [i32, C.POINTER(vp)]
    lib.pca_ctx_destroy.argtypes = [vp]
    lib.pca_ctx_destroy.restype = None
    lib.pca_last_error.argtypes = [vp]
    lib.pca_last_error.restype = C.c_char_p
    lib.pca_status.argtypes = [vp, vp, C.POINTER(C.c_uint32)]
    lib.pca_status_peek.argtypes = [vp, C.POINTER(C.c_uint32)]
    lib.pca_status_mirror.argtypes = [vp]
    lib.pca_status_mirror.restype = vp
    lib.pca_kitti_project_sample_filter.argtypes = [
        vp, C.POINTER(PcaKittiFrame), i32, C.POINTER(C.c_double), i32, i32, C.POINTER(C.c_uint64),
        C.POINTER(PcaStore), vp, i32, vp
    ]
    lib.pca_kitti_project_sample_filter_ex.argtypes = [
        vp, C.POINTER(PcaKittiFrame), i32, C.POINTER(C.c_double), i32, i32, C.POINTER(C.c_uint64),
        C.POINTER(PcaStore), vp, i32, i32, vp
    ]
    lib.pca_nusc_sample_filter_transform_ex.argtypes = [
        vp, vp, vp, C.c_int32, vp, vp, i32, i32, i32, C.POINTER(C.c_double), C.POINTER(C.c_uint64),
        C.POINTER(PcaStore), vp, i32, i32, vp
    ]
    lib.pca_nusc_sample_filter_transform_batch.argtypes = [
        vp, C.POINTER(PcaNuscFrame), i32, i32, i32, i32, C.POINTER(C.c_uint64), C.POINTER(PcaStore), vp, i32, i32, vp
    ]
    lib.pca_sample_bilinear.argtypes = [vp, vp, i32, i32, vp, C.c_int32, vp, vp]
    lib.pca_nusc_sample_filter_transform.argtypes = [
        vp, vp, vp, C.c_int32, vp, vp, i32, i32, i32, C.POINTER(C.c_double), C.POINTER(C.c_uint64),
        C.POINTER(PcaStore), vp, i32, vp
    ]
    lib.pca_nusc_project_cams.argtypes = [
        vp, vp, C.c_int32, C.POINTER(C.c_double), C.POINTER(C.c_double), C.POINTER(C.c_double),
        C.POINTER(C.c_double), C.POINTER(C.c_double), i32, vp, vp, vp, vp
    ]
    lib.pca_nusc_merge_sweeps_workspace_bytes.argtypes = [i64, i32]
    lib.pca_nusc_merge_sweeps_workspace_bytes.restype = i64
    lib.pca_nusc_merge_sweeps.argtypes = [vp, vp, i64, vp, i32, vp, i32, C.c_float, C.c_double, vp, i64, vp, vp, vp]
    lib.pca_retransform.argtypes = [vp, C.POINTER(PcaStore), vp, i32, i32, C.POINTER(C.c_double), i32, vp]
    lib.pca_retransform_batch_tail.argtypes = [vp, C.POINTER(PcaStore), vp, i32, i32, C.POINTER(C.c_double), vp]
    lib.pca_mark_dynamic.argtypes = [vp, C.POINTER(PcaStore), vp, C.POINTER(C.c_int32), C.POINTER(C.c_int32), i32, vp]
    lib.pca_bev_workspace_bytes.argtypes = [i64, i32]
    lib.pca_bev_workspace_bytes.restype = i64
    lib.pca_bev_generate.argtypes = [
        vp, C.POINTER(PcaStore), vp, vp, i32, i32, i32, i64, C.POINTER(PcaBevParams), C.POINTER(C.c_double), i32,
        vp, i64, vp, vp, vp
    ]
    lib.pca_bev_generate_ex.argtypes = [
        vp, C.POINTER(PcaStore), vp, vp, i32, i32, i32, i64, C.POINTER(PcaBevParams), C.POINTER(C.c_double), i32,
        vp, i64, vp, vp, vp, vp
    ]
    lib.pca_image_to_nchw_f32.argtypes = [vp, vp, i32, i32, C.POINTER(C.c_float), C.POINTER(C.c_float), vp, vp]
    a = list(lib.pca_bev_generate_ex.argtypes)
    lib.pca_bev_generate_chain.argtypes = a[:9] + [vp, vp, i32, i32] + a[11:]
    lib.pca_bev_generate_many.argtypes = [vp, C.POINTER(PcaStore), vp, vp, C.POINTER(PcaBevJob), i32, i64, vp, i64, vp]
    lib.pca_bev_class_workspace_bytes.argtypes = [i64, i32]
    lib.pca_bev_class_workspace_bytes.restype = i64
    lib.pca_bev_class_planes.argtypes = [vp, C.POINTER(PcaStore), vp, i32, i32, i32, i64, C.POINTER(PcaBevParams),
                                         C.POINTER(PcaClassGroup), i32, vp, vp, i32, vp, i64, vp, vp, vp, vp]
    lib.pca_bev_elev_workspace_bytes.argtypes = [i64, i32]
    lib.pca_bev_elev_workspace_bytes.restype = i64
    lib.pca_bev_elev_partition.argtypes = [vp, C.POINTER(PcaStore), vp, i32, i32, i64, C.POINTER(PcaBevParams), C.c_double, i32,
                                           vp, vp, i32, vp, i64, vp, vp, vp, vp, vp]
    lib.pca_bev_warp.argtypes = [vp, vp, vp, i32, i32, C.c_double, C.c_double, C.c_double, C.c_double, vp]
    lib.pca_voxel_dedup_workspace_bytes.restype = C.c_int64
    lib.pca_voxel_dedup_workspace_bytes.argtypes = [i64, i32]
    lib.pca_voxel_dedup.argtypes = [vp, C.POINTER(PcaStore), vp, i32, i32, C.c_double, i64, vp, i64, vp]
    lib.pca_icp_workspace_bytes.restype = C.c_int64
    lib.pca_icp_workspace_bytes.argtypes = [i32]
    lib.pca_icp_register.argtypes = [vp, vp, i32, vp, i32, C.c_double, C.POINTER(C.c_double), i32, C.c_double,
                                     C.c_double, vp, i64, C.POINTER(C.c_double), C.POINTER(C.c_double),
                                     C.POINTER(C.c_double), C.POINTER(C.c_int), vp]
    lib.pca_host_ego_to_grid.argtypes = [vp, i32, vp, C.c_double, C.c_double, C.c_double, i32, vp, vp]
    lib.pca_lanes_workspace_bytes.argtypes = [i64, i32, i64]
    lib.pca_lanes_workspace_bytes.restype = i64
    lib.pca_lanes_transform.argtypes = [vp, vp, i64, vp, vp]
    lib.pca_lanes_to_grid.argtypes = [vp, vp, vp, vp, i64, C.c_int32, vp, i32, i64, vp, vp, vp, vp, vp]
    dp = C.POINTER(C.c_double)
    lib.pca_host_gemv4_probe.argtypes = [vp, i32, vp, vp, i64, vp]
    lib.pca_host_gemv4_mode.argtypes = [i32]
    lib.pca_host_incr_probe.argtypes = [vp, vp, i64, i64, i64, vp]
    lib.pca_host_incr_blocks.argtypes = [i32]
    lib.pca_host_track_create.argtypes = [C.POINTER(vp), vp]
    lib.pca_host_track_destroy.argtypes = [vp]
    lib.pca_host_track_destroy.restype = None
    for name in ('pca_host_track_len', 'pca_host_track_n_segments'):
        getattr(lib, name).argtypes = [vp]
        getattr(lib, name).restype = i64
    for name in ('pca_host_track_poses', 'pca_host_track_segments'):
        getattr(lib, name).argtypes = [vp]
        getattr(lib, name).restype = vp
    lib.pca_host_track_set.argtypes = [vp, vp, i64, vp, i64]
    lib.pca_host_track_transform.argtypes = [vp, vp]
    lib.pca_host_track_append.argtypes = [vp, vp]
    lib.pca_host_track_push_segment.argtypes = [vp, dp]
    lib.pca_host_track_incr.argtypes = [vp, vp]
    lib.pca_host_track_evict_beyond.argtypes = [vp, C.c_double, C.c_double]
    lib.pca_host_track_evict_beyond.restype = i64
    lib.pca_host_track_step.argtypes = [vp, vp, C.c_double, dp]
    lib.pca_host_track_step.restype = i64
    lib.pca_host_track_trigger.argtypes = [vp, C.c_double, i64, C.c_double]
    lib.pca_host_track_trigger.restype = i64
    lib.pca_host_stage_h2d.argtypes = [i32, vp, vp, vp, vp, vp]
    lib.pca_host_d2h_async.argtypes = [vp, vp, vp, i64, vp]
    lib.pca_host_d2h_wait.argtypes = [vp, i32]
    lib.pca_deflate_workspace_bytes.argtypes = [i64]
    lib.pca_deflate_workspace_bytes.restype = i64
    lib.pca_deflate_chunks.argtypes = [vp, vp, vp, i64, vp, vp, vp, vp, vp]
    lib.pca_deflate_chunks_dyn.argtypes = [vp, vp, vp, i64, vp, vp, vp, vp, vp]
    lib.pca_host_crc32_combine.argtypes = [C.c_uint32, C.c_uint32, i64]
    lib.pca_host_crc32_combine.restype = C.c_uint32
    lib.pca_host_gzip_assemble.argtypes = [i32, vp, vp, vp, vp, vp, i64]
    lib.pca_host_gzip_assemble.restype = i64
    lib.pca_kitti_integrate.argtypes = [vp, C.POINTER(PcaKittiObs), C.POINTER(C.c_double), i32, i32, C.POINTER(C.c_uint64),
                                        C.POINTER(PcaStore), vp, i32, i32, vp, vp, C.c_double, C.POINTER(C.c_int64),
                                        C.POINTER(C.c_double), vp]
    lib.pca_kitti_generate_bev.argtypes = [vp, C.POINTER(PcaStore), vp, i32, i32, i32, i64, C.POINTER(PcaBevParams), vp, vp,
                                           i32, i32, vp, i64, vp, vp, vp, vp, vp, C.POINTER(C.c_int32), vp]
    lib.pca_host_camera_cone.argtypes = [vp, i32, i32, vp]
    lib.pca_host_camera_cone.restype = None
    lib.pca_host_view_hull.argtypes = [i32, vp, vp, vp, vp, vp, C.POINTER(C.c_int), C.POINTER(C.c_int)]
    lib.pca_bev_bin_range.argtypes = [vp, i32, i32]
    lib.pca_bev_view_hint.argtypes = [vp, i32, i32, vp, vp, vp, vp, vp]
    lib.pca_f32_box_decode.argtypes = [vp, i32, vp]
    lib.pca_f32_box_decode.restype = None
    lib.pca_debug_bev_level1.argtypes = [vp, vp]
    lib.pca_debug_icp_layout.argtypes = [i32, i32, C.POINTER(C.c_int64)]
    lib.pca_kitti_integrate_v.argtypes = [vp, vp]
    lib.pca_kitti_generate_bev_v.argtypes = [vp, vp]
    lib.pca_k1_defer.argtypes = [vp, i32]
    lib.pca_k1_flush.argtypes = [vp]
    lib.pca_profile_enable.argtypes = [vp, i32]
    lib.pca_profile_read.argtypes = [vp, i32, C.POINTER(C.c_double), C.POINTER(C.c_int64)]
    _lib = lib
    return lib


class Context:

    _by_device = {}
    _raw_stream = None
    _tls = threading.local()

    def __init__(self, device_index):
        import torch
        if not torch.cuda.is_available():
            raise RuntimeError('pca_amd needs an AMD GPU (torch.cuda.is_available() is False); '
                               'there is no CPU fallback')
        self.lib = load()
        self.device_index = int(device_index)
        h = C.c_void_p()
        if self.lib.pca_ctx_create(self.device_index, C.byref(h)) != 0:
            raise RuntimeError('pca_ctx_create failed')
        self.h = h
        self._mirror = (C.c_uint32 * 8).from_address(self.lib.pca_status_mirror(h))
        self._mirror_q = (C.c_uint64 * 4).from_address(C.addressof(self._mirror))

    @classmethod
    def get(cls, device=None):
        import torch
        if not torch.cuda.is_available():
            raise RuntimeError('pca_amd needs an AMD GPU (torch.cuda.is_available() is False); '
                               'there is no CPU fallback')
        idx = torch.cuda.current_device() if device is None else torch.device(device).index or 0
        lane = getattr(cls._tls, 'lane', None)
        if lane is not None and lane.device_index == idx:
            return lane
        if idx not in cls._by_device:
            cls._by_device[idx] = Context(idx)
        return cls._by_device[idx]

    def destroy(self):
        if self.h is not None:
            self.lib.pca_ctx_destroy(self.h)
            self.h = None

    def stream(self):
        return C.c_void_p(self.stream_int())

    def stream_int(self):
        raw = self._raw_stream
        if raw is None:
            import torch
            raw = getattr(torch._C, '_cuda_getCurrentRawStream', None)
            if raw is None:
                return torch.cuda.current_stream(self.device_index).cuda_stream
            self._raw_stream = raw
        return raw(self.device_index)

    def check(self, rc):
        if rc != 0:
            raise RuntimeError('pca: ' + self.lib.pca_last_error(self.h).decode())

    def profile(self, on):
        self.check(self.lib.pca_profile_enable(self.h, int(on)))

    def profile_read(self):
        out = {}
        for k, name in enumerate(KERNEL_IDS):
            ms, n = C.c_double(0), C.c_int64(0)
            self.check(self.lib.pca_profile_read(self.h, k, C.byref(ms), C.byref(n)))
            out[name] = (ms.value, n.value)
        return out

    def peek_status(self):
        q = self._mirror_q
        if not (q[0] | q[1] | q[2] | q[3]):
            return 0
        m = self._mirror
        return sum(1 << b for b in range(8) if m[b])

    def check_status(self):
        st = self.status()
        if not st:
            return
        said = [(STATUS_UV_OUT_OF_IMAGE, AssertionError, 'pts_uv must be all inside image'),
                (STATUS_STORE_OVERFLOW, RuntimeError, 'pca: device point store overflow (points were dropped)'),
                (STATUS_LOOKBACK_TIMEOUT, RuntimeError,
                 'pca: a compaction workgroup timed out waiting for its predecessor (output invalid)'),
                (STATUS_NEGATIVE_INTENSITY, ValueError, 'pca: negative lidar intensity on the f32 path (pass intensity64 to bev())'),
                (STATUS_LANES_BISECT_CAP, RuntimeError, 'pca: a lane\'s border crossing was not found within the iteration cap (row invalid)')]
        hit = [(exc, msg) for bit, exc, msg in said if st & bit]
        rest = st & ~(STATUS_UV_OUT_OF_IMAGE | STATUS_STORE_OVERFLOW | STATUS_LOOKBACK_TIMEOUT | STATUS_NEGATIVE_INTENSITY | STATUS_LANES_BISECT_CAP)
        if rest:
            hit.append((RuntimeError, 'pca: unknown device status bits 0x%x' % rest))
        raise hit[0][0]('; '.join(msg for _, msg in hit))

    def poll_status(self):
        if self.peek_status():
            self.check_status()

    def status(self):
        st = C.c_uint32(0)
        self.check(self.lib.pca_status(self.h, self.stream(), C.byref(st)))
        return st.value


class Lane:

    def __init__(self, device=None, priority=0):
        import torch
        idx = torch.cuda.current_device() if device is None else torch.device(device).index or 0
        self.ctx = Context(idx)
        self.stream = torch.cuda.Stream(device=idx, priority=priority)
        self._guard = None
        self._outer = None

    def __enter__(self):
        import torch
        self._outer = getattr(Context._tls, 'lane', None)
        Context._tls.lane = self.ctx
        self._guard = torch.cuda.stream(self.stream)
        self._guard.__enter__()
        return self

    def __exit__(self, *exc):
        self._guard.__exit__(*exc)
        Context._tls.lane = self._outer
        self._guard = None
        return False

    def synchronize(self):
        self.stream.synchronize()

    def close(self):
        self.stream.synchronize()
        self.ctx.destroy()
```

### pc-accumulation-lib_amd/pca_amd/device_store.py

```python
import ctypes as C
import os

import numpy as np
import torch

from . import _lib
from ._lib import PcaBevParams, PcaKittiFrame, PcaStore

CULL = os.environ.get('PCA_BEV_CULL', '1') != '0'


class DeviceStore:
    CHAIN_MAX = 4
    CHAIN_K = int(os.environ.get('PCA_BEV_CHAIN', '4'))

    def __init__(self, capacity=1 << 24, max_frames=4096, device=None, intensity_div255=False):
        self.ctx = _lib.Context.get(device)
        self.device = torch.device('cuda', self.ctx.device_index)
        self.intensity_div255 = bool(intensity_div255)
        self.max_frames = int(max_frames)
        self._alloc(int(capacity))
        self.frame_off = torch.zeros(self.max_frames + 1, dtype=torch.int64, device=self.device)
        self._moved = np.eye(4)
        self.cull = CULL
        self.hints_taken = 0
        self._alloc_frame_tables(self.max_frames)
        self.head = 0
        self.tail = 0
        self.ub_tail = 0
        self.lb_head = 0
        self._ub = []
        self._ub_sum = 0
        self._pending = []
        self._k1_cache = None
        self._k1_src = None
        self._ia = None
        self._ws = None
        self._ws_many = None
        self._ws_points, self._ws_px = 0, 0
        self._ws_side = {}
        self._dedup_ws = None
        self._obs_out = None
        self._k1_noted = None
        self._pend_T = (C.c_double * (16 * self.CHAIN_MAX))()
        self._pend_T_np = np.frombuffer(self._pend_T, dtype=np.float64)
        self._pend_ends = (C.c_int * self.CHAIN_MAX)()

    def _alloc(self, cap):
        d = self.device
        self.capacity = cap
        self._cstore = None
        self.x = torch.empty(cap, dtype=torch.float64, device=d)
        self.y = torch.empty(cap, dtype=torch.float64, device=d)
        self.z = torch.empty(cap, dtype=torch.float64, device=d)
        self.intensity = torch.empty(cap, dtype=torch.float32, device=d)
        self.rgbs = torch.empty(cap, dtype=torch.int32, device=d)
        self.inst = torch.empty(cap, dtype=torch.int32, device=d)
        self.dyn = torch.empty(cap, dtype=torch.uint8, device=d)

    def _arrays(self):
        return (self.x, self.y, self.z, self.intensity, self.rgbs, self.inst, self.dyn)

    BOX_EVERY = 16

    def _alloc_frame_tables(self, max_frames, keep=None):
        n1 = max_frames + 1
        box = torch.zeros((n1, 6), dtype=torch.int32, device=self.device)
        then = np.full((n1, 12), np.nan)
        seen = np.tile(np.array([1, -1] * 3, dtype=np.float32), (n1, 1))
        cone = np.zeros(n1, dtype=bool)
        if keep is not None:
            a, n = keep
            box[:n] = self.frame_box[a:a + n]
            then[:n], seen[:n], cone[:n] = self._then[a:a + n], self._box[a:a + n], self._has_cone[a:a + n]
        self.frame_box, self._then, self._box, self._has_cone = box, then, seen, cone
        self._then_addr, self._box_addr = then.ctypes.data, seen.ctypes.data
        self._box_pin = None
        self._box_copy = None
        self._since_box = 0
        self._cone = None
        self._n_nocone = 0 if keep is None else int(np.count_nonzero(~cone[:keep[1]] & np.isfinite(then[:keep[1], 0])))
        self._cstore = None

    def _note_moved(self, Ts):
        for T in Ts:
            M = T.reshape(4, 4) @ self._moved
            M[3] = (0., 0., 0., 1.)
            self._moved = M

    def _note_frame(self, slot, cone_key):
        self._then[slot] = self._moved[:3].reshape(12)
        if cone_key is not None:
            if self._cone is None or self._cone[0] != cone_key:
                if self._cone is not None:
                    self._has_cone[self.head:self.tail] = False
                    self._n_nocone = self.tail - self.head
                out = np.empty(15)
                Pm = np.frombuffer(cone_key[0], dtype=np.float64)
                self.ctx.lib.pca_host_camera_cone(Pm.ctypes.data, int(cone_key[1]), int(cone_key[2]), out.ctypes.data)
                self._cone = (cone_key, out, out.ctypes.data)
            self._has_cone[slot] = True
        else:
            self._n_nocone += 1
        self._since_box += 1
        self._poll_boxes()
        if self._since_box >= self.BOX_EVERY and self._box_copy is None:
            n = self.tail - self.head
            if n > 0:
                if self._box_pin is None or self._box_pin.shape[0] < self.frame_box.shape[0]:
                    self._box_pin = torch.empty(tuple(self.frame_box.shape), dtype=torch.int32, pin_memory=True)
                self._box_pin[:n].copy_(self.frame_box[self.head:self.tail], non_blocking=True)
                ev = torch.cuda.Event()
                ev.record()
                self._box_copy = (ev, self.head, n)
                self._since_box = 0

    def _poll_boxes(self):
        if self._box_copy is None or not self._box_copy[0].query():
            return
        _, first, n = self._box_copy
        self._box_copy = None
        rows = self._box_pin[:n].numpy()
        dec = np.empty((n, 6), dtype=np.float32)
        self.ctx.lib.pca_f32_box_decode(rows.ctypes.data, n, dec.ctypes.data)
        known = dec[:, 0] <= dec[:, 1]
        tgt = self._box[first:first + n]
        tgt[known] = dec[known]

    def view_hint_into(self, args, first_frame, last_frame):
        n = last_frame - first_frame
        if not self.cull or n < 4:
            return 0
        a = self.head + first_frame
        args.hint_slot0 = a
        args.hint_then, args.hint_box = self._then_addr + 96 * a, self._box_addr + 24 * a
        args.hint_cone = self._cone[2] if (self._cone is not None and self._n_nocone == 0) else None
        args.hint_now = self._moved.ctypes.data
        return n

    def view_hint(self, prm, first_frame, last_frame, write_back):
        n = last_frame - first_frame
        if not self.cull or write_back or n < 4:
            return 0
        a = self.head + first_frame
        cone = self._cone[2] if (self._cone is not None and self._n_nocone == 0) else None
        return self._count_hint(self.ctx.lib.pca_bev_view_hint(self.ctx.h, a, n, self._then_addr + 96 * a, self._box_addr + 24 * a, cone,
                                              self._moved.ctypes.data, C.addressof(prm)))

    def _count_hint(self, r):
        self.hints_taken += 1 if r > 0 else 0
        return r

    def c_store(self):
        if self._cstore is None:
            self._cstore = PcaStore(self.x.data_ptr(), self.y.data_ptr(), self.z.data_ptr(), self.intensity.data_ptr(),
                                    self.rgbs.data_ptr(), self.inst.data_ptr(), self.dyn.data_ptr(), self.capacity,
                                    self.frame_box.data_ptr())
        return self._cstore

    @property
    def n_frames(self):
        return self.tail - self.head

    def set_defer_k1(self, on):
        self.ctx.check(self.ctx.lib.pca_k1_defer(self.ctx.h, 1 if on else 0))
        self.ctx.k1_defer = bool(on)
        if not on:
            self._k1_noted = None

    def flush_k1(self):
        if self._k1_noted is not None:
            self.ctx.check(self.ctx.lib.pca_k1_flush(self.ctx.h))
            self._k1_noted = None

    def __del__(self):
        try:
            if self._k1_noted is not None:
                self.flush_k1()
        except Exception:
            pass

    def offsets(self):
        self.flush_k1()
        off = self.frame_off[self.head:self.tail + 1].cpu().numpy()
        self.lb_head = int(off[0])
        self.ub_tail = int(off[-1])
        self._ub = [int(v) for v in np.diff(off)]
        self._ub_sum = sum(self._ub)
        return off

    def sizes(self):
        return np.diff(self.offsets())

    def poll_status(self):
        self.ctx.poll_status()

    def check_status(self):
        self.ctx.check_status()

    def reserve(self, n_new, n_slots=1):
        if self.tail + n_slots <= self.max_frames and self.ub_tail + n_new <= self.capacity:
            return
        self.flush_pending()
        off = self.offsets()
        a, b = int(off[0]), int(off[-1])
        live, nf = b - a, self.n_frames
        new_cap = self.capacity
        while live + n_new > new_cap:
            new_cap *= 2
        new_maxf = self.max_frames
        while nf + n_slots > new_maxf:
            new_maxf *= 2
        old = self._arrays()
        if new_cap != self.capacity:
            self._alloc(new_cap)
            for dst, src in zip(self._arrays(), old):
                dst[:live] = src[a:b]
        elif a > 0:
            for t in old:
                t[:live] = t[a:b].clone()
        self.max_frames = new_maxf
        new_off = torch.zeros(new_maxf + 1, dtype=torch.int64, device=self.device)
        new_off[:nf + 1] = torch.from_numpy(off - a).to(self.device)
        self.frame_off = new_off
        cone = self._cone
        self._alloc_frame_tables(new_maxf, keep=(self.head, nf))
        self._cone = cone
        self.head, self.tail = 0, nf
        self.lb_head, self.ub_tail = 0, live

    def evict(self, k):
        k = int(k)
        if self._n_nocone and k:
            sl = slice(self.head, self.head + k)
            self._n_nocone -= int(np.count_nonzero(~self._has_cone[sl] & np.isfinite(self._then[sl, 0])))
        self.head += k
        self._ub_sum -= sum(self._ub[:int(k)])
        del self._ub[:int(k)]

    def max_window_points(self):
        return max(self._ub_sum, 1)

    def clear(self):
        self.flush_k1()
        self.head = self.tail = 0
        self.ub_tail = self.lb_head = 0
        self._ub = []
        self._ub_sum = 0
        self._pending = []
        self.frame_off.zero_()
        self._alloc_frame_tables(self.max_frames)
        self._moved = np.eye(4)

    @staticmethod
    def kitti_descs(frames):
        descs = (PcaKittiFrame * len(frames))()
        for k, f in enumerate(frames):
            n = int(f['pts'].shape[0])
            assert f['pts'].dtype == torch.float32 and f['pts'].is_contiguous()
            descs[k].pts = f['pts'].data_ptr() if n else None
            descs[k].rgb = f['rgb'].data_ptr() if f.get('rgb') is not None else None
            descs[k].sem = f['sem'].data_ptr() if f.get('sem') is not None else None
            descs[k].sem_gt = f['sem_gt'].data_ptr() if f.get('sem_gt') is not None else None
            descs[k].n = n
        return descs

    def append_kitti(self, frames, P, H, W, filters, descs=None, sample_mode='nearest'):
        lib, ctx = self.ctx.lib, self.ctx
        n_in = sum(int(f['pts'].shape[0]) for f in frames)
        self.reserve(n_in, len(frames))
        if descs is None:
            descs = self.kitti_descs(frames)
        st = self.c_store()
        key = (np.asarray(P, dtype=np.float64).tobytes(), tuple(int(c) for c in (filters or ())))
        if self._k1_cache is None or self._k1_cache[0] != key:
            self._k1_cache = (key, _lib.f64_array(P, 12), _lib.class_mask(filters))
        Pc, fmask = self._k1_cache[1], self._k1_cache[2]
        ctx.check(lib.pca_kitti_project_sample_filter_ex(ctx.h, descs, len(frames), Pc, int(H), int(W),
                                                         fmask, C.byref(st), self.frame_off.data_ptr(), self.tail,
                                                         _lib.SAMPLE_MODES[sample_mode], ctx.stream()))
        self.tail += len(frames)
        self.ub_tail += n_in
        self._ub += [int(f['pts'].shape[0]) for f in frames]
        self._ub_sum += n_in

    def append_kitti_obs(self, obs, P, H, W, filters, sample_mode='nearest', track=None, T_new_prev=None, horizon=0., keep=None):
        lib, ctx = self.ctx.lib, self.ctx
        n = int(obs.n)
        self.reserve(n, 1)
        src = self._k1_src
        if src is not None and src[0] is P and src[1] is filters and P.tobytes() == src[2] and tuple(filters or ()) == src[3]:
            key = self._k1_cache[0]
        else:
            key = (np.asarray(P, dtype=np.float64).tobytes(), tuple(int(c) for c in (filters or ())))
            ok = isinstance(P, np.ndarray) and P.dtype == np.float64 and all(type(c) is int for c in (filters or ()))
            self._k1_src = (P, filters, key[0], key[1]) if ok else None
        if self._k1_cache is None or self._k1_cache[0] != key:
            self._k1_cache = (key, _lib.f64_array(P, 12), _lib.class_mask(filters))
        Pc, fmask = self._k1_cache[1], self._k1_cache[2]
        st = self.c_store()
        th = getattr(track, '_h', None)
        a = self._ia
        if a is None:
            a = self._ia = _lib.PcaKittiIntegrateArgs()
            self._ia_T = np.zeros(16)
            self._ia_T_addr = self._ia_T.ctypes.data
            self._ia_const = None
        const = (id(obs), id(Pc), int(H), int(W), id(st), id(self.frame_off), sample_mode, th, float(horizon))
        if const != self._ia_const:
            a.obs, a.P, a.H, a.W, a.filter_mask = C.addressof(obs), C.addressof(Pc), int(H), int(W), C.addressof(fmask)
            a.store, a.frame_off, a.sample_mode = C.addressof(st), self.frame_off.data_ptr(), _lib.SAMPLE_MODES[sample_mode]
            a.track, a.horizon = getattr(th, 'value', th), float(horizon)
            self._ia_const = const
            self._ia_keep = (obs, Pc, fmask, st, self.frame_off)
        a.slot = self.tail
        if th is not None:
            self._ia_T[:] = np.asarray(T_new_prev, dtype=np.float64).reshape(16)
            a.T_new_prev = self._ia_T_addr
        else:
            a.T_new_prev = None
        a.stream = ctx.stream_int() or None
        ctx.check(lib.pca_kitti_integrate_v(ctx.h, C.addressof(a)))
        self._k1_noted = (keep, ) if getattr(ctx, 'k1_defer', False) else None
        self._note_frame(self.tail, (key[0], int(H), int(W)) if obs.sem_gt is None else None)
        self.tail += 1
        self.ub_tail += n
        self._ub.append(n)
        self._ub_sum += n
        if th is None:
            return None, None
        v = a.path_length
        return int(a.evicted), (None if v != v else np.float64(v))

    def append_nusc(self, pc, cam_idx, imgs, sems, T, filters, sample_mode='nearest'):
        lib, ctx = self.ctx.lib, self.ctx
        n = int(pc.shape[0])
        self.reserve(n)
        ncam, H, W = sems.shape
        st = self.c_store()
        ctx.check(lib.pca_nusc_sample_filter_transform_ex(ctx.h, pc.data_ptr(), cam_idx.data_ptr(), n, imgs.data_ptr(),
                                                          sems.data_ptr(), int(ncam), int(H), int(W),
                                                          _lib.f64_array(T, 16), _lib.class_mask(filters),
                                                          C.byref(st), self.frame_off.data_ptr(), self.tail,
                                                          _lib.SAMPLE_MODES[sample_mode], ctx.stream()))
        self.tail += 1
        self.ub_tail += n
        self._ub.append(n)
        self._ub_sum += n

    def append_nusc_many(self, frames, filters, sample_mode='nearest'):
        lib, ctx = self.ctx.lib, self.ctx
        if not frames:
            return
        ncam, H, W = (int(v) for v in frames[0]['sems'].shape)
        max_tiles = 16384
        b0 = 0
        while b0 < len(frames):
            tiles, b1 = 0, b0
            while b1 < len(frames):
                t = max((int(frames[b1]['pc'].shape[0]) + 511) // 512, 1)
                if b1 > b0 and tiles + t > max_tiles:
                    break
                tiles += t
                b1 += 1
            part = frames[b0:b1]
            n_in = sum(int(f['pc'].shape[0]) for f in part)
            self.reserve(n_in, len(part))
            descs = (_lib.PcaNuscFrame * len(part))()
            keep = []
            for k, f in enumerate(part):
                assert f['pc'].dtype == torch.float64 and f['pc'].is_contiguous() and f['cam_idx'].dtype == torch.int64
                assert tuple(f['sems'].shape) == (ncam, H, W) and f['imgs'].is_contiguous() and f['sems'].is_contiguous()
                n = int(f['pc'].shape[0])
                Tc = _lib.f64_array(f['T'], 16)
                keep.append(Tc)
                descs[k].pc = f['pc'].data_ptr() if n else None
                descs[k].cam_idx = f['cam_idx'].data_ptr() if n else None
                descs[k].imgs, descs[k].sems = f['imgs'].data_ptr(), f['sems'].data_ptr()
                descs[k].n = n
                descs[k].T = C.cast(Tc, C.POINTER(C.c_double))
            st = self.c_store()
            ctx.check(lib.pca_nusc_sample_filter_transform_batch(ctx.h, descs, len(part), ncam, H, W, _lib.class_mask(filters),
                                                                 C.byref(st), self.frame_off.data_ptr(), self.tail,
                                                                 _lib.SAMPLE_MODES[sample_mode], ctx.stream()))
            self.tail += len(part)
            self.ub_tail += n_in
            self._ub += [int(f['pc'].shape[0]) for f in part]
            self._ub_sum += n_in
            b0 = b1

    def retransform(self, Ts, defer=False):
        if self.n_frames == 0:
            return
        Ts = np.ascontiguousarray(Ts, dtype=np.float64).reshape(-1, 16)
        self._note_moved(Ts)
        if defer and Ts.shape[0] == 1:
            if len(self._pending) >= self.CHAIN_MAX:
                self.flush_pending()
            self._pending.append((Ts[0].copy(), self.tail))
            return
        self.flush_pending()
        self._launch_retransform(Ts, self.head, self.tail)

    def _launch_retransform(self, Ts, begin_slot, end_slot):
        st = self.c_store()
        ctx = self.ctx
        ctx.check(ctx.lib.pca_retransform(ctx.h, C.byref(st), self.frame_off.data_ptr(), begin_slot, end_slot,
                                          _lib.f64_array(Ts, Ts.size), Ts.shape[0], ctx.stream()))

    def retransform_batch(self, Ts, n_new):
        Ts = np.ascontiguousarray(Ts, dtype=np.float64).reshape(-1, 16)
        assert Ts.shape[0] == n_new
        self.flush_pending()
        self._note_moved(Ts)
        first_new = self.tail - n_new
        if first_new > self.head:
            st, ctx = self.c_store(), self.ctx
            ctx.check(ctx.lib.pca_retransform(ctx.h, C.byref(st), self.frame_off.data_ptr(), self.head, first_new,
                                              _lib.f64_array(Ts, Ts.size), Ts.shape[0], ctx.stream()))
        st, ctx = self.c_store(), self.ctx
        ctx.check(ctx.lib.pca_retransform_batch_tail(ctx.h, C.byref(st), self.frame_off.data_ptr(), first_new, n_new,
                                                     _lib.f64_array(Ts, Ts.size), ctx.stream()))

    def flush_pending(self):
        pend, self._pending = self._pending, []
        begin = self.head
        for k, (_, end_slot) in enumerate(pend):
            if end_slot > begin:
                self._launch_retransform(np.stack([T for T, _ in pend[k:]]), begin, end_slot)
                begin = end_slot

    def mark_dynamic(self, pairs):
        pairs = list(pairs)
        if not pairs:
            return
        slots = (C.c_int32 * len(pairs))(*[self.head + int(f) for f, _ in pairs])
        insts = (C.c_int32 * len(pairs))(*[int(i) for _, i in pairs])
        st = self.c_store()
        ctx = self.ctx
        ctx.check(ctx.lib.pca_mark_dynamic(ctx.h, C.byref(st), self.frame_off.data_ptr(), slots, insts, len(pairs),
                                           ctx.stream()))

    def voxel_dedup(self, voxel_size):
        if self.n_frames == 0:
            return
        self.flush_pending()
        ctx, lib = self.ctx, self.ctx.lib
        max_points = self.max_window_points()
        need = lib.pca_voxel_dedup_workspace_bytes(max_points, self.n_frames)
        if self._dedup_ws is None or self._dedup_ws.numel() < need:
            self._dedup_ws = torch.empty(int(need) + 256, dtype=torch.uint8, device=self.device)
        st = self.c_store()
        ctx.check(lib.pca_voxel_dedup(ctx.h, C.byref(st), self.frame_off.data_ptr(), self.head, self.tail,
                                      float(voxel_size), max_points, self._dedup_ws.data_ptr(),
                                      self._dedup_ws.numel(), ctx.stream()))

    def bev(self, split_frame, prm, want_f64=False, intensity64=None, first_frame=0, last_frame=None, out16=None,
            extra=None):
        ctx, lib = self.ctx, self.ctx.lib
        last_frame = self.n_frames if last_frame is None else last_frame
        px = int(prm.px)
        max_points = self.bev_workspace(px)
        if out16 is not None:
            assert out16.dtype == torch.float16 and out16.is_contiguous() and tuple(out16.shape) == (21, px, px)
        p16 = out16 if out16 is not None else torch.empty((21, px, px), dtype=torch.float16, device=self.device)
        p64 = torch.empty((21, px, px), dtype=torch.float64, device=self.device) if want_f64 else None
        st = self.c_store()
        n_pend, pend_T, pend_ends, write_back = self.bev_pending(first_frame, last_frame)
        if extra is not None:
            assert extra.dtype == torch.float64 and extra.is_contiguous() \
                and tuple(extra.shape) == (3, len(_lib.BEV_EXTRA_PLANES), px, px)
        self.view_hint(prm, first_frame, last_frame, n_pend > 0 and write_back)
        ctx.check(lib.pca_bev_generate_chain(ctx.h, C.byref(st), None if intensity64 is None else intensity64.data_ptr(),
                                             self.frame_off.data_ptr(), self.head + first_frame, self.head + split_frame,
                                             self.head + last_frame, max_points, C.byref(prm), pend_T, pend_ends, n_pend,
                                             write_back, self._ws.data_ptr(), self._ws.numel(),
                                             None if p64 is None else p64.data_ptr(), p16.data_ptr(),
                                             None if extra is None else extra.data_ptr(), ctx.stream()))
        self.bev_done(write_back)
        return p16, p64

    def bev_workspace(self, px):
        max_points = self.max_window_points()
        if self._ws is None or max_points > self._ws_points or px != self._ws_px:
            self._ws_points, self._ws_px = int(max_points * 1.25) + 1, px
            need = self.ctx.lib.pca_bev_workspace_bytes(self._ws_points, px)
            if self._ws is None or self._ws.numel() < need:
                self._ws = torch.empty(int(need) + 256, dtype=torch.uint8, device=self.device)
        return max_points

    def bev_pending(self, first_frame, last_frame):
        if not self._pending:
            return 0, None, None, 1
        if first_frame != 0 or self._pending[-1][1] > self.head + last_frame:
            self.flush_pending()
            return 0, None, None, 1
        n_pend = 0
        for T, e in self._pending:
            if e > self.head:
                self._pend_T_np[16 * n_pend:16 * n_pend + 16] = T
                self._pend_ends[n_pend] = int(e)
                n_pend += 1
        if n_pend == 0:
            return 0, None, None, 0
        return n_pend, self._pend_T, self._pend_ends, (1 if n_pend >= self.CHAIN_K else 0)

    def bev_done(self, write_back):
        if self._pending and write_back:
            self._pending = []
        self._k1_noted = None

    def _side_workspace(self, name, workspace_bytes, max_points, px):
        ws = self._ws_side.setdefault(name, [None, 0, 0])
        if ws[0] is None or max_points > ws[1] or px != ws[2]:
            ws[1], ws[2] = int(max_points * 1.25) + 1, px
        need = workspace_bytes(ws[1], px)
        if ws[0] is None or ws[0].numel() < need:
            ws[0] = torch.empty(int(need) + 256, dtype=torch.uint8, device=self.device)
        return ws[0]

    def bev_class_planes(self, split_frame, prm, groups, first_frame=0, last_frame=None, want_counts=False):
        ctx, lib = self.ctx, self.ctx.lib
        self.flush_k1()
        last_frame = self.n_frames if last_frame is None else last_frame
        px, ng = int(prm.px), len(groups)
        cg = (_lib.PcaClassGroup * max(ng, 1))()
        for k, g in enumerate(groups):
            cg[k].mask[:] = list(_lib.class_mask(g))
        n_pend, pend_T, pend_ends, _ = self.bev_pending(first_frame, last_frame)
        max_points = self.max_window_points()
        ws = self._side_workspace('class', lib.pca_bev_class_workspace_bytes, max_points, px)
        shape = (3, max(ng, 1), max(px, 1), max(px, 1))
        p16 = torch.empty(shape, dtype=torch.float16, device=self.device)
        p64 = torch.empty(shape, dtype=torch.float64, device=self.device)
        cnt = torch.empty((3, shape[1] + 1) + shape[2:], dtype=torch.int32, device=self.device) if want_counts else None
        st = self.c_store()
        ctx.check(lib.pca_bev_class_planes(ctx.h, C.byref(st), self.frame_off.data_ptr(), self.head + first_frame,
                                           self.head + split_frame, self.head + last_frame, max_points, C.byref(prm), cg, ng,
                                           pend_T, pend_ends, n_pend, ws.data_ptr(), ws.numel(),
                                           p64.data_ptr(), p16.data_ptr(), None if cnt is None else cnt.data_ptr(),
                                           ctx.stream()))
        return p16, p64, cnt

    def bev_elev_partition(self, prm, elev_thresh, first_frame=0, last_frame=None, include_dyn=False, mark_dyn=False,
                           max_points=None):
        ctx, lib = self.ctx, self.ctx.lib
        last_frame = self.n_frames if last_frame is None else last_frame
        px = int(prm.px)
        if mark_dyn:
            self.flush_pending()
        n_pend, pend_T, pend_ends, _ = self.bev_pending(first_frame, last_frame)
        bound = self.max_window_points()
        max_points = bound if max_points is None else max(int(max_points), 1)
        ws = self._side_workspace('elev', lib.pca_bev_elev_workspace_bytes, max_points, px)
        side = max(px, 1)
        elev = torch.empty((side, side), dtype=torch.float64, device=self.device)
        obs = torch.empty((side, side), dtype=torch.uint8, device=self.device)
        flags = torch.empty(max_points, dtype=torch.uint8, device=self.device)
        counts = torch.empty(3, dtype=torch.int64, device=self.device)
        st = self.c_store()
        ctx.check(lib.pca_bev_elev_partition(ctx.h, C.byref(st), self.frame_off.data_ptr(), self.head + first_frame,
                                             self.head + last_frame, max_points, C.byref(prm), float(elev_thresh),
                                             1 if include_dyn else 0, pend_T, pend_ends, n_pend, ws.data_ptr(),
                                             ws.numel(), elev.data_ptr(), obs.data_ptr(), flags.data_ptr(),
                                             counts.data_ptr(), ctx.stream()))
        self._k1_noted = None
        lo_hi = self.frame_off[[self.head + first_frame, self.head + last_frame]].cpu()
        lo, n = int(lo_hi[0]), min(int(lo_hi[1] - lo_hi[0]), max_points)
        flags = flags[:n]
        if mark_dyn:
            self.dyn[lo + torch.nonzero(flags == 1).squeeze(1)] = 1
        return {'elev': elev, 'observed': obs.bool(), 'flags': flags, 'counts': counts}

    def bev_many(self, jobs, out16):
        ctx, lib = self.ctx, self.ctx.lib
        n = len(jobs)
        if n == 0:
            return out16
        self.flush_pending()
        px = int(jobs[0][1].px)
        assert out16.dtype == torch.float16 and out16.is_contiguous() and tuple(out16.shape) == (n, 21, px, px)
        max_points = self.max_window_points()
        per = (int(lib.pca_bev_workspace_bytes(max_points, px)) + 255) & ~255
        need = per * n + 512
        if self._ws_many is None or self._ws_many.numel() < need:
            self._ws_many = torch.empty(int(need * 1.25), dtype=torch.uint8, device=self.device)
        cj = (_lib.PcaBevJob * n)()
        plane_bytes = 21 * px * px * 2
        for k, (split, prm, first, last) in enumerate(jobs):
            last = self.n_frames if last is None else last
            cj[k].slot_begin, cj[k].slot_split, cj[k].slot_end = self.head + first, self.head + split, self.head + last
            C.memmove(C.addressof(cj[k].prm), C.addressof(prm), C.sizeof(PcaBevParams))
            cj[k].planes = None
            cj[k].planes_f16 = out16.data_ptr() + k * plane_bytes
        st = self.c_store()
        ctx.check(lib.pca_bev_generate_many(ctx.h, C.byref(st), None, self.frame_off.data_ptr(), cj, n, max_points,
                                            self._ws_many.data_ptr(), self._ws_many.numel(), ctx.stream()))
        return out16

    def rows(self, frame=None):
        self.flush_pending()
        off = self.offsets()
        lo, hi = (int(off[0]), int(off[-1])) if frame is None else (int(off[frame]), int(off[frame + 1]))
        out = np.empty((hi - lo, 10))
        out[:, 0] = self.x[lo:hi].cpu().numpy()
        out[:, 1] = self.y[lo:hi].cpu().numpy()
        out[:, 2] = self.z[lo:hi].cpu().numpy()
        i = self.intensity[lo:hi].cpu().numpy().astype(np.float64)
        out[:, 3] = i / 255. if self.intensity_div255 else i
        r = self.rgbs[lo:hi].cpu().numpy().view(np.uint32)
        out[:, 4], out[:, 5], out[:, 6], out[:, 7] = r & 255, (r >> 8) & 255, (r >> 16) & 255, r >> 24
        out[:, 8] = self.inst[lo:hi].cpu().numpy()
        out[:, 9] = self.dyn[lo:hi].cpu().numpy()
        return out

    def frame_rows(self):
        off = self.offsets()
        allrows = self.rows()
        base = int(off[0])
        return [allrows[int(off[k]) - base:int(off[k + 1]) - base] for k in range(self.n_frames)]

    def load_rows(self, rows_list, intensity64_out=None):
        self.clear()
        total = int(sum(r.shape[0] for r in rows_list))
        if total > self.capacity or len(rows_list) > self.max_frames:
            self.max_frames = max(self.max_frames, len(rows_list))
            self._alloc(max(total, 1))
            self.frame_off = torch.zeros(self.max_frames + 1, dtype=torch.int64, device=self.device)
            self._alloc_frame_tables(self.max_frames)
        rows = np.concatenate([np.asarray(r, dtype=np.float64).reshape(-1, 10) for r in rows_list]) if rows_list \
            else np.zeros((0, 10))
        c = rows[:, 4:8]
        if rows.size and not (np.all(c == np.floor(c)) and c.min() >= 0 and c.max() <= 255):
            raise NotImplementedError('rgb / semantic columns must hold integers 0..255')
        if rows.size and not np.all(rows[:, 8] == np.floor(rows[:, 8])):
            raise NotImplementedError('instance column must hold integers')
        d = self.device
        self.x[:total] = torch.from_numpy(np.ascontiguousarray(rows[:, 0])).to(d)
        self.y[:total] = torch.from_numpy(np.ascontiguousarray(rows[:, 1])).to(d)
        self.z[:total] = torch.from_numpy(np.ascontiguousarray(rows[:, 2])).to(d)
        inten = rows[:, 3]
        raw = np.rint(inten * 255.) if self.intensity_div255 else inten
        raw32 = raw.astype(np.float32)
        back = raw32.astype(np.float64) / 255. if self.intensity_div255 else raw32.astype(np.float64)
        i64 = None
        if not np.array_equal(back, inten) or (inten.size and (inten.min() < 0 or np.signbit(inten).any())):
            i64 = torch.from_numpy(np.ascontiguousarray(inten)).to(d)
        self.intensity[:total] = torch.from_numpy(raw32).to(d)
        cu = c.astype(np.uint32)
        packed = (cu[:, 0] | (cu[:, 1] << 8) | (cu[:, 2] << 16) | (cu[:, 3] << 24)).astype(np.uint32)
        self.rgbs[:total] = torch.from_numpy(packed.view(np.int32)).to(d)
        self.inst[:total] = torch.from_numpy(rows[:, 8].astype(np.int32)).to(d)
        self.dyn[:total] = torch.from_numpy((rows[:, 9] == 1).astype(np.uint8)).to(d)
        off = np.concatenate([[0], np.cumsum([r.shape[0] for r in rows_list])]).astype(np.int64)
        self.frame_off[:off.size] = torch.from_numpy(off).to(d)
        self.head, self.tail = 0, len(rows_list)
        self.lb_head, self.ub_tail = 0, total
        self._ub = [int(r.shape[0]) for r in rows_list]
        self._ub_sum = sum(self._ub)
        return i64


def make_bev_params(origin, R, dx, dy, view, px, height_filter, int_scaler, int_sep_scaler, int_mid_threshold,
                    road_class, dynobj_classes, intensity_div255, rgb_fill=0.):
    prm = PcaBevParams()
    prm.origin[:] = [float(v) for v in origin]
    prm.R[:] = [float(v) for v in np.asarray(R, dtype=np.float64).ravel()]
    prm.dx, prm.dy, prm.view = float(dx), float(dy), float(view)
    prm.height_filter = float('nan') if height_filter is None else float(height_filter)
    prm.int_scaler = float(int_scaler)
    prm.int_sep_scaler = float(int_sep_scaler)
    prm.int_mid_threshold = float(int_mid_threshold)
    prm.rgb_fill = float(rgb_fill)
    prm.px = int(px)
    prm.road_class = int(road_class)
    prm.dynobj_mask[:] = list(_lib.class_mask(dynobj_classes))
    prm.intensity_div255 = int(bool(intensity_div255))
    return prm
```

### pc-accumulation-lib_amd/pca_amd/host_logic.py

```python
import math
import random
from collections.abc import Sequence

import numpy as np


def pose_dist(p0, p1):
    return np.sqrt(np.sum((p1 - p0)**2))


_TRI = {}


def incremental_path_dists(seg_dists):
    d = np.array(seg_dists)
    n = len(d)
    tri = _TRI.get(n)
    if tri is None:
        if len(_TRI) > 64:
            _TRI.clear()
        tri = _TRI[n] = np.tri(n)
    return np.matmul(tri, d)


class ArrayList(Sequence):

    def __init__(self, arr):
        self._a = arr

    def __len__(self):
        return self._a.shape[0]

    def __getitem__(self, i):
        return self._a[i].tolist()

    def __iter__(self):
        return iter(self._a.tolist())

    def __array__(self, dtype=None, copy=None):
        return np.array(self._a, dtype=dtype)

    def tolist(self):
        return self._a.tolist()

    def __eq__(self, other):
        return self._a.tolist() == (other.tolist() if isinstance(other, (ArrayList, np.ndarray)) else other)

    def __repr__(self):
        return repr(self._a.tolist())


class NumpyPoseTrack:

    def __init__(self):
        self._H = np.zeros((0, 4, 1))
        self._D = np.zeros(0)

    @property
    def _P(self):
        return self._H[:, :3, 0]

    @property
    def seg_dists(self):
        return ArrayList(self._D.copy())

    @seg_dists.setter
    def seg_dists(self, value):
        self._D = np.array(value, dtype=np.float64).reshape(-1)

    def seg_array(self):
        return self._D

    @property
    def poses(self):
        return ArrayList(self._P.copy())

    @poses.setter
    def poses(self, value):
        P = np.array(value, dtype=np.float64).reshape(-1, 3)
        self._H = np.ones((P.shape[0], 4, 1))
        self._H[:, :3, 0] = P

    def __len__(self):
        return self._H.shape[0]

    def pose(self, idx):
        return self._P[idx].copy()

    def as_array(self):
        return self._P.copy()

    def apply_transform(self, T):
        if self._H.shape[0] == 0:
            return
        H = np.matmul(T, self._H)
        H[:, 3, 0] = 1.0
        self._H = H

    def append(self, pose):
        h = np.ones((1, 4, 1))
        h[0, :3, 0] = np.asarray(pose, dtype=np.float64).reshape(3)
        self._H = np.concatenate([self._H, h])

    def push_segment(self):
        self._D = np.append(self._D, pose_dist(self._H[-1, :3, 0], self._H[-2, :3, 0]))
        return np.sum(self._D)

    def evict_beyond(self, horizon_dist, path_length):
        if not path_length > horizon_dist:
            return 0
        incr = incremental_path_dists(self._D)
        incr -= path_length - horizon_dist
        k = int((incr > 0.).argmax())
        self._H = self._H[k:]
        self._D = self._D[k:]
        return k

    def incr(self):
        return incremental_path_dists(self._D)

    def step(self, T_new_prev, horizon_dist):
        if len(self) > 0:
            self.apply_transform(T_new_prev)
        self.append([0., 0., 0.])
        if len(self) < 2:
            return 0, None
        path_length = self.push_segment()
        return self.evict_beyond(horizon_dist, path_length), path_length

    def trigger(self, bev_horizon, previous_idx, min_step):
        if len(self) < 2:
            return None
        d = self.incr()
        if d[-1] < bev_horizon:
            return None
        present_idx = int(((d - bev_horizon) > 0).argmax())
        if d[-1] - d[present_idx] < bev_horizon:
            return None
        if pose_dist(self.pose(previous_idx), self.pose(present_idx)) < min_step:
            return None
        return present_idx


def _numpy_gemv_entry():
    import ctypes as C
    try:
        from threadpoolctl import threadpool_info
        paths = [p['filepath'] for p in threadpool_info() if p.get('user_api') == 'blas' and p.get('filepath')]
    except Exception:
        return None
    for path in paths:
        try:
            blas = C.CDLL(path)
        except OSError:
            continue
        for sym in ('scipy_cblas_dgemv64_', 'cblas_dgemv64_'):
            fn = getattr(blas, sym, None)
            if fn is not None:
                return C.cast(fn, C.c_void_p).value, blas
    return None


class CPoseTrack:
    _lib = None
    _gemv = None
    _blas = None

    def __init__(self):
        import ctypes as C
        self._C = C
        h = C.c_void_p()
        if self._lib.pca_host_track_create(C.byref(h), self._gemv) != 0:
            raise RuntimeError('pca_host_track_create failed')
        self._h = h
        self._pl = C.c_double(0.0)
        self._win = None

    def __del__(self):
        try:
            self._lib.pca_host_track_destroy(self._h)
        except Exception:
            pass

    def __len__(self):
        return self._lib.pca_host_track_len(self._h)

    def _view(self, ptr, n, width):
        if n == 0:
            return np.zeros((0, width)) if width > 1 else np.zeros(0)
        a = np.ctypeslib.as_array((self._C.c_double * (n * width)).from_address(ptr))
        return a.reshape(n, width) if width > 1 else a

    def as_array(self):
        n = len(self)
        return self._view(self._lib.pca_host_track_poses(self._h), n, 4)[:, :3].copy()

    def poses_window(self, first, last):
        n = len(self)
        ptr = self._lib.pca_host_track_poses(self._h)
        c = self._win
        if c is None or c[0] != ptr or c[1] < n:
            c = self._win = (ptr, n, self._view(ptr, n, 4))
        return c[2][first:last, :3].copy()

    def pose(self, idx):
        n = len(self)
        i = int(idx)
        if i < 0:
            i += n
        if not 0 <= i < n:
            raise IndexError('pose index out of range')
        return self._view(self._lib.pca_host_track_poses(self._h), n, 4)[i, :3].copy()

    def seg_array(self):
        nd = self._lib.pca_host_track_n_segments(self._h)
        return self._view(self._lib.pca_host_track_segments(self._h), nd, 1).copy()

    @property
    def poses(self):
        return ArrayList(self.as_array())

    @poses.setter
    def poses(self, value):
        P = np.ascontiguousarray(np.array(value, dtype=np.float64).reshape(-1, 3))
        D = self.seg_array()
        self._lib.pca_host_track_set(self._h, P.ctypes.data, P.shape[0], D.ctypes.data, D.shape[0])

    @property
    def seg_dists(self):
        return ArrayList(self.seg_array())

    @seg_dists.setter
    def seg_dists(self, value):
        D = np.ascontiguousarray(np.array(value, dtype=np.float64).reshape(-1))
        P = np.ascontiguousarray(self.as_array())
        self._lib.pca_host_track_set(self._h, P.ctypes.data, P.shape[0], D.ctypes.data, D.shape[0])

    def apply_transform(self, T):
        T = np.ascontiguousarray(T, dtype=np.float64)
        self._lib.pca_host_track_transform(self._h, T.ctypes.data)

    def append(self, pose):
        p = np.ascontiguousarray(np.asarray(pose, dtype=np.float64).reshape(3))
        self._lib.pca_host_track_append(self._h, p.ctypes.data)

    def push_segment(self):
        if self._lib.pca_host_track_push_segment(self._h, self._C.byref(self._pl)) != 0:
            raise IndexError('push_segment needs two poses')
        return np.float64(self._pl.value)

    def evict_beyond(self, horizon_dist, path_length):
        return int(self._lib.pca_host_track_evict_beyond(self._h, float(horizon_dist), float(path_length)))

    def incr(self):
        out = np.empty(self._lib.pca_host_track_n_segments(self._h))
        self._lib.pca_host_track_incr(self._h, out.ctypes.data)
        return out

    def step(self, T_new_prev, horizon_dist):
        T = np.ascontiguousarray(T_new_prev, dtype=np.float64)
        k = self._lib.pca_host_track_step(self._h, T.ctypes.data, float(horizon_dist), self._C.byref(self._pl))
        pl = self._pl.value
        return int(k), (None if pl != pl else np.float64(pl))

    def trigger(self, bev_horizon, previous_idx, min_step):
        k = self._lib.pca_host_track_trigger(self._h, float(bev_horizon), int(previous_idx), float(min_step))
        if k == -2:
            raise IndexError('pose index out of range')
        return None if k < 0 else int(k)


def _bind_c_track():
    import os
    if os.environ.get('PCA_HOST_TRACK', 'c') == 'numpy':
        return None
    lib = _c_library()
    entry = _numpy_gemv_entry()
    if lib is None or entry is None or not hasattr(lib, 'pca_host_track_step'):
        return None
    CPoseTrack._lib, CPoseTrack._gemv, CPoseTrack._blas = lib, entry[0], entry[1]
    rng = np.random.default_rng(20261004)
    n = 4096
    Tm = rng.normal(size=(n, 4, 4)) * rng.choice([1e-3, 1., 1e3], size=(n, 1, 1))
    Tm[::3, 3] = [0., 0., 0., 1.]
    X = np.ones((n, 4, 1))
    X[:, :3, 0] = rng.normal(size=(n, 3)) * rng.choice([1e-2, 1., 1e2, 1e4], size=(n, 1))
    want = np.concatenate([np.matmul(Tm[i], X[i:i + 1]) for i in range(n)])[:, :, 0]
    got = np.empty((n, 4))
    lib.pca_host_gemv4_mode(0)
    for mode in (1, 2, 3, 4, 5):
        lib.pca_host_gemv4_probe(entry[0], mode, Tm.ctypes.data, np.ascontiguousarray(X[:, :, 0]).ctypes.data, n, got.ctypes.data)
        if np.array_equal(got, want):
            lib.pca_host_gemv4_mode(mode)
            break
    lib.pca_host_incr_blocks(0)
    ok = True
    for n in (2, 7, 8, 9, 63, 64, 65, 127, 200, 201, 255, 333, 512, 1000):
        d = np.ascontiguousarray(rng.uniform(0.2, 1.7, n))
        want = np.matmul(np.tri(n), d)
        out = np.empty(8)
        for r0 in sorted({0, 8 * ((n - 1) // 8), 8 * (n // 16), 8 * (n // 24)}):
            r1 = min(r0 + 8, n)
            lib.pca_host_incr_probe(entry[0], d.ctypes.data, n, r0, r1, out.ctypes.data)
            ok = ok and np.array_equal(out[:r1 - r0], want[r0:r1])
    lib.pca_host_incr_blocks(1 if ok else 0)
    a, b = CPoseTrack(), NumpyPoseTrack()
    prev = 0
    for f in range(160):
        ang = rng.uniform(-0.05, 0.05)
        T = np.eye(4)
        T[:2, :2] = [[np.cos(ang), -np.sin(ang)], [np.sin(ang), np.cos(ang)]]
        T[:3, 3] = rng.uniform(-1.5, 0.5, 3) * [1.0, 0.05, 0.01]
        ra, rb = a.step(T, 37.5), b.step(T, 37.5)
        prev -= ra[0]
        ta, tb = (a.trigger(11.0, prev, 1.0), b.trigger(11.0, prev, 1.0)) if -len(b) <= prev < len(b) else (None, None)
        if ra != rb or ta != tb or not np.array_equal(a.as_array(), b.as_array()) \
                or not np.array_equal(a.seg_array(), b.seg_array()) or not np.array_equal(a.incr(), b.incr()):
            return None
        if ta is not None:
            prev = ta
    return CPoseTrack


_TRACK_CLASS = []


def PoseTrack():
    if not _TRACK_CLASS:
        try:
            _TRACK_CLASS.append(_bind_c_track() or NumpyPoseTrack)
        except Exception:
            _TRACK_CLASS.append(NumpyPoseTrack)
    return _TRACK_CLASS[0]()


def rotation_matrix_3d(ang):
    c, s = np.cos(ang), np.sin(ang)
    return np.array([[c, -s, 0], [s, c, 0], [0, 0, 1]])


def heading_rot_ang(ego_traj_present):
    ang = 0.5 * np.pi
    if len(ego_traj_present) > 1:
        dx = ego_traj_present[-1][0] - ego_traj_present[-2][0]
        dy = ego_traj_present[-1][1] - ego_traj_present[-2][1]
        ang += np.arctan2(dy, dx)
    return np.pi - ang


def pos2grid_inplace(mat, view, px):
    mat[:, 0:2] = np.floor(mat[:, 0:2] / view * px + 0.5 * px)
    return mat


def _inside(x, y, b0x, b0y, b1x, b1y):
    return (b0x < x and x < b1x) and (b0y < y and y < b1y)


def bisect_box_crossing(x0, y0, x1, y1, bbox, thresh=1e-4):
    x0, y0, x1, y1 = float(x0), float(y0), float(x1), float(y1)
    b0x, b0y, b1x, b1y = (float(b) for b in bbox)
    gap = math.inf
    iters = 0
    xm = ym = 0.0
    while gap > thresh:
        xm = 0.5 * (x0 + x1)
        ym = 0.5 * (y0 + y1)
        p0_in = (b0x < x0 and x0 < b1x) and (b0y < y0 and y0 < b1y)
        mid_in = (b0x < xm and xm < b1x) and (b0y < ym and ym < b1y)
        if mid_in == p0_in:
            gap = math.sqrt((xm - x0)**2 + (ym - y0)**2)
            x0, y0 = xm, ym
        else:
            gap = math.sqrt((xm - x1)**2 + (ym - y1)**2)
            x1, y1 = xm, ym
        iters += 1
    return xm, ym, iters


def crop_trajectory(traj, view, thresh=1e-4):
    n = traj.shape[0]
    if n < 2:
        return np.zeros((0, 3))
    h = 0.5 * view
    lo = -h
    x, y = traj[:, 0], traj[:, 1]
    inside = (lo < x) & (x < h) & (lo < y) & (y < h)
    a_in, b_in = inside[:-1], inside[1:]
    crossing = a_in != b_in
    per_edge = a_in.astype(np.int64) + crossing.astype(np.int64)
    total = int(per_edge.sum())
    if total == 0:
        return np.zeros((0, 3))
    start = np.cumsum(per_edge) - per_edge
    out = np.empty((total, 3))
    ka = np.nonzero(a_in)[0]
    out[start[ka]] = traj[ka, :3]
    bbox = [lo, lo, h, h]
    for k in np.nonzero(crossing)[0]:
        ix, iy, _ = bisect_box_crossing(traj[k, 0], traj[k, 1], traj[k + 1, 0], traj[k + 1, 1], bbox, thresh)
        out[start[k] + (1 if a_in[k] else 0)] = (ix, iy, traj[k, 2])
    return out


def _crop_edges(traj, view, thresh=1e-4):
    n = traj.shape[0]
    if n < 2:
        return np.zeros((0, 3)), np.zeros(max(n, 1), dtype=np.int64)
    h = 0.5 * view
    lo = -h
    x, y = traj[:, 0], traj[:, 1]
    inside = (lo < x) & (x < h) & (lo < y) & (y < h)
    a_in, b_in = inside[:-1], inside[1:]
    crossing = a_in != b_in
    per_edge = a_in.astype(np.int64) + crossing.astype(np.int64)
    start = np.concatenate([[0], np.cumsum(per_edge)])
    out = np.empty((int(start[-1]), 3))
    ka = np.nonzero(a_in)[0]
    out[start[ka]] = traj[ka, :3]
    bbox = [lo, lo, h, h]
    for k in np.nonzero(crossing)[0]:
        ix, iy, _ = bisect_box_crossing(traj[k, 0], traj[k, 1], traj[k + 1, 0], traj[k + 1, 1], bbox, thresh)
        out[start[k] + (1 if a_in[k] else 0)] = (ix, iy, traj[k, 2])
    return out, start


_CLIB = []


def _c_library():
    if not _CLIB:
        try:
            from . import _lib
            _CLIB.append(_lib.load())
        except Exception:
            _CLIB.append(None)
    return _CLIB[0]


def transform_ego_split(full, split, rot_mat, dx, dy, view, px):
    t = np.array(full, dtype=np.float64)
    n = t.shape[0]
    lib = _c_library()
    if lib is not None and t.ndim == 2 and t.shape[1] == 3:
        R = np.ascontiguousarray(rot_mat, dtype=np.float64)
        rows = np.empty((max(2 * (n - 1), 1), 3))
        start = np.zeros(max(n, 1), dtype=np.int32)
        m = lib.pca_host_ego_to_grid(t.ctypes.data, n, R.ctypes.data, float(dx), float(dy), float(view), int(px),
                                     rows.ctypes.data, start.ctypes.data)
        rows = rows[:m]
    else:
        t[:, :3] = np.matmul(rot_mat, t[:, :3].T).T
        t[:, 0] += dx
        t[:, 1] += dy
        rows, start = _crop_edges(t, view)
        rows = pos2grid_inplace(rows, view, px)
    empty = np.zeros((0, 3))
    e_p = max(split - 1, 0)
    present = rows[:start[e_p]].copy() if split >= 2 else empty
    future = rows[start[split]:].copy() if n - split >= 2 else empty
    return present, future, rows


def transform_traj(traj, rot_mat, dx, dy, view, px, mutate=True):
    if not mutate:
        lib = _c_library()
        if lib is not None and isinstance(traj, np.ndarray) and traj.ndim == 2 and traj.shape[1] == 3:
            t = np.ascontiguousarray(traj, dtype=np.float64)
            n = t.shape[0]
            if n < 2:
                return np.zeros((0, 3))
            R = np.ascontiguousarray(rot_mat, dtype=np.float64)
            rows = np.empty((2 * (n - 1), 3))
            start = np.empty(n, dtype=np.int32)
            m = lib.pca_host_ego_to_grid(t.ctypes.data, n, R.ctypes.data, float(dx), float(dy), float(view), int(px),
                                         rows.ctypes.data, start.ctypes.data)
            return rows[:m]
    traj[:, :3] = np.matmul(rot_mat, traj[:, :3].T).T
    traj[:, 0] += dx
    traj[:, 1] += dy
    return pos2grid_inplace(crop_trajectory(traj, view), view, px)


def cal_warp_params(idx_0, idx_1, idx_max):
    a_1 = (idx_1 - idx_0**2 / idx_max) / (idx_0 * (1.0 - idx_0 / idx_max))
    a_2 = (1.0 - a_1) / idx_max
    return (a_1, a_2)


def get_random_warp_params(mean_ratio, max_ratio, I, J):
    max_val = max_ratio * (I / 2.0)
    mean_val = mean_ratio * max_val
    i_warp = np.random.normal(mean_val, max_val)
    j_warp = np.random.normal(mean_val, max_val)
    if abs(i_warp) > max_val:
        i_warp = max_val
    if abs(j_warp) > max_val:
        j_warp = max_val
    if random.random() < 0.5:
        i_warp = -i_warp
    if random.random() < 0.5:
        j_warp = -j_warp
    return (int(I / 2) + i_warp, int(J / 2) + j_warp)


def warp_source_index(coef_1, coef_2, n):
    k = np.arange(n, dtype=np.float64)
    src = np.rint(coef_1 * k + coef_2 * (k * k)).astype(np.int64)
    return np.clip(src, 0, n - 1)


def warp_dense_probmaps(maps, a_1, a_2, b_1, b_2):
    _, I, J = maps.shape
    i_src = warp_source_index(a_1, a_2, I)
    j_src = warp_source_index(b_1, b_2, J)
    out = np.zeros(maps.shape)
    out[:, :J, :I] = maps[:, j_src[:, None], i_src[None, :]]
    return out


def warp_point(x, y, a_1, a_2, b_1, b_2, I, J):
    if math.isclose(a_2, 0.0, abs_tol=1e-6):
        xw = x
    else:
        xw = int(np.rint((-a_1 + np.sqrt(a_1**2 + 4.0 * a_2 * x)) / (2 * a_2)))
    if math.isclose(b_2, 0.0, abs_tol=1e-6):
        yw = y
    else:
        yw = int(np.rint((-b_1 + np.sqrt(b_1**2 + 4.0 * b_2 * y)) / (2 * b_2)))
    xw = 0 if xw < 0 else (I - 1 if xw >= I else xw)
    yw = 0 if yw < 0 else (J - 1 if yw >= J else yw)
    return (xw, yw)


def warp_sparse_points(pnts, a_1, a_2, j_warp, j_mid, px):
    b_1r, b_2r = cal_warp_params(px - j_warp, j_mid, px - 1)
    for k in range(pnts.shape[0]):
        xw, yw = warp_point(pnts[k, 0], pnts[k, 1], a_1, a_2, b_1r, b_2r, px, px)
        pnts[k, 0] = xw
        pnts[k, 1] = yw
    return pnts
```

Measured before the change: 1583 Mpoints/s.

## Move per-frame step bookkeeping and BEV view setup into a native state block

Adds a C step-state block that keeps the moved transform, per-frame tables, owed transform chain and view parameters (origin, heading rotation). New integrate_s and generate_bev_s entry points consume this block, so Python no longer rebuilds the track transform, pending chain and raster params on every frame. A startup probe checks the C heading and rotation against numpy bit for bit and falls back to numpy if they differ. This targets Python and ctypes host overhead per frame, at the cost of more duplicated state that must stay in sync between Python and C.

```diff
diff --git a/include/pca.h b/include/pca.h
--- a/include/pca.h
+++ b/include/pca.h
@@ -269,6 +269,22 @@
     int32_t hinted, pad2;
 } pca_kitti_generate_bev_args;
 int pca_kitti_generate_bev_v(pca_ctx *ctx, pca_kitti_generate_bev_args *a);
+
+typedef struct {
+    double *moved; double *then; uint8_t *has_cone; const float *box; double *pend_T; int32_t *pend_ends; const double *cone;
+    int32_t slots, chain_k, cull, prm_ready;
+    int32_t head, tail, split, pend_n;
+    int64_t n_nocone;
+    double view, ang, dxy[2];
+    int32_t hinted, n_rows, write_back, n_pending;
+} pca_kitti_step_state;
+int pca_host_step_state_note(pca_kitti_step_state *s, const double *T , int flags);
+int pca_host_step_state_view(pca_kitti_step_state *s, const pca_host_track *track, pca_bev_params *prm,
+                             double *chain_T , int32_t *chain_ends );
+int pca_host_step_state_last_step(pca_kitti_step_state *s, const pca_host_track *track);
+int pca_host_heading_probe(const double *dxdy , int64_t n, int ang_given, double *ang , double *R );
+int pca_kitti_integrate_s(pca_ctx *ctx, pca_kitti_integrate_args *a, pca_kitti_step_state *s, int flags);
+int pca_kitti_generate_bev_s(pca_ctx *ctx, pca_kitti_generate_bev_args *a, pca_kitti_step_state *s);
 
 int pca_host_stage_h2d(int n, const void *const *src, void *const *pinned, void *const *dev, const int64_t *bytes,
                        void *stream);
diff --git a/pc-accumulation-lib_amd/bev_generator/bev_generator.py b/pc-accumulation-lib_amd/bev_generator/bev_generator.py
--- a/pc-accumulation-lib_amd/bev_generator/bev_generator.py
+++ b/pc-accumulation-lib_amd/bev_generator/bev_generator.py
@@ -117,6 +117,16 @@
         return BEVGenerator._RasterBatch(self)
 
     def _raster_params(self, origin, rot_mat, dx, dy, aug_view_size, intensity_div255):
+        prm = self._raster_block(intensity_div255)
+        head = self._tmp.get(id(prm))
+        if head is None:
+            head = self._tmp[id(prm)] = np.frombuffer((ctypes.c_double * 15).from_address(ctypes.addressof(prm)), dtype=np.float64)
+        head[0:3] = origin
+        head[3:12] = np.asarray(rot_mat, dtype=np.float64).reshape(9)
+        head[12], head[13], head[14] = dx, dy, aug_view_size
+        return prm
+
+    def _raster_block(self, intensity_div255):
         key = ('prm', bool(intensity_div255), self.pixel_size, self.height_filter, self.int_scaler,
                self.int_sep_scaler, self.int_mid_threshold, getattr(self, 'rgb_fill', 0))
         prm = self._tmp.get(key)
@@ -128,12 +138,6 @@
                                                    self.height_filter, self.int_scaler, self.int_sep_scaler,
                                                    self.int_mid_threshold, sem_idxs.get('road', -1), dyn_cls,
                                                    intensity_div255, getattr(self, 'rgb_fill', 0))
-        head = self._tmp.get(id(prm))
-        if head is None:
-            head = self._tmp[id(prm)] = np.frombuffer((ctypes.c_double * 15).from_address(ctypes.addressof(prm)), dtype=np.float64)
-        head[0:3] = origin
-        head[3:12] = np.asarray(rot_mat, dtype=np.float64).reshape(9)
-        head[12], head[13], head[14] = dx, dy, aug_view_size
         return prm
 
     def _tmp_store(self, key):
diff --git a/pc-accumulation-lib_amd/csrc/pca_api.hip b/pc-accumulation-lib_amd/csrc/pca_api.hip
--- a/pc-accumulation-lib_amd/csrc/pca_api.hip
+++ b/pc-accumulation-lib_amd/csrc/pca_api.hip
@@ -175,6 +175,7 @@
                       const pca_bev_params *prm)
 {
     if (!ctx) return -1;
+    ctx->bin_valid = false;
     int first = 0, last = 0;
     if (pca_host_view_hull(F, then, box, cone, now, prm, &first, &last)) return -1;
     if (first == 0 && last == F - 1) return 0;
diff --git a/pc-accumulation-lib_amd/csrc/pca_session.hip b/pc-accumulation-lib_amd/csrc/pca_session.hip
--- a/pc-accumulation-lib_amd/csrc/pca_session.hip
+++ b/pc-accumulation-lib_amd/csrc/pca_session.hip
@@ -1,6 +1,7 @@
 #include <vector>
 
 #include "pca_common.h"
+#include "pca_step_state.h"
 
 int pca_stage_copy(const void *const *src, void *const *dst, const int64_t *bytes, int n);
 
@@ -14,6 +15,8 @@
     if (!ctx) return -1;
     if (!obs || obs->n < 0 || !P || !filter_mask || !store || !frame_off) { ctx->err = "kitti_integrate: bad arguments"; return -1; }
     if (track && (!T_new_prev || !evicted || !path_length)) { ctx->err = "kitti_integrate: the pose track needs T_new_prev and its outputs"; return -1; }
+    if (H < 0 || W < 0 || (int64_t)H * W * 3 >= (1ll << 31)) { ctx->err = "k1: image too large"; return -1; }
+    if (obs->n > 0 && !obs->pts) { ctx->err = "k1: bad frame"; return -1; }
     hipStream_t s = (hipStream_t)stream;
     PCA_CHECK(ctx, hipSetDevice(ctx->device));
     if (pca_k1_flush_pending(ctx)) return -1;
@@ -96,9 +99,9 @@
                            double *traj_rows, int32_t *traj_start, int32_t *n_rows, void *stream)
 {
     if (!ctx) return -1;
-    if (!prm || !planes_f16 || !track || !traj_rows || !traj_start || !n_rows) { ctx->err = "kitti_generate_bev: bad arguments"; return -1; }
+    if (!prm || !planes_f16 || !track || !traj_rows || !traj_start || !n_rows) { ctx->bin_valid = false; ctx->err = "kitti_generate_bev: bad arguments"; return -1; }
     const int64_t F = pca_host_track_len(track);
-    if (F != slot_end - slot_begin) { ctx->err = "kitti_generate_bev: the pose track and the window disagree about the number of frames"; return -1; }
+    if (F != slot_end - slot_begin) { ctx->bin_valid = false; ctx->err = "kitti_generate_bev: the pose track and the window disagree about the number of frames"; return -1; }
     static thread_local std::vector<double> rel;
     rel.resize((size_t)(3 * (F > 0 ? F : 1)));
     const double *Hp = pca_host_track_poses(track);
@@ -124,6 +127,7 @@
 int pca_kitti_generate_bev_v(pca_ctx *ctx, pca_kitti_generate_bev_args *a)
 {
     if (!ctx) return -1;
+    ctx->bin_valid = false;
     if (!a) { ctx->err = "kitti_generate_bev_v: no argument block"; return -1; }
     a->hinted = 0;
     if (a->hint_F > 0 && !(a->n_pending > 0 && a->write_back)) {
@@ -137,4 +141,72 @@
                                   &a->n_rows, a->stream);
 }
 
-}
+int pca_host_step_state_note(pca_kitti_step_state *s, const double *T, int flags) { return pca_ss_note(s, T, flags); }
+
+int pca_host_step_state_view(pca_kitti_step_state *s, const pca_host_track *track, pca_bev_params *prm, double *chain_T,
+                             int32_t *chain_ends)
+{
+    if (!s || !track || !prm || !chain_T || !chain_ends || !s->pend_T || !s->pend_ends) return -1;
+    if (s->head < 0 || s->tail < s->head || s->tail > s->slots) return -1;
+    if (s->prm_ready != 1 &&
+        pca_ss_view_head(pca_host_track_poses(track), pca_host_track_len(track), (int64_t)s->split - s->head, s->view,
+                         s->prm_ready == 2 ? &s->ang : nullptr, prm))
+        return -1;
+    const int n = pca_ss_chain(s, chain_T, chain_ends, &s->write_back);
+    if (n < 0) return -1;
+    s->n_pending = n;
+    return 0;
+}
+
+int pca_host_step_state_last_step(pca_kitti_step_state *s, const pca_host_track *track)
+{
+    if (!s || !track) return -1;
+    return pca_ss_last_step(pca_host_track_poses(track), pca_host_track_len(track), (int64_t)s->split - s->head, s->dxy);
+}
+
+int pca_host_heading_probe(const double *dxdy, int64_t n, int ang_given, double *ang, double *R)
+{
+    if (!dxdy || !ang || !R || n < 0) return -1;
+    for (int64_t i = 0; i < n; ++i) {
+        if (!ang_given) ang[i] = pca_ss_heading(1, dxdy[2 * i], dxdy[2 * i + 1]);
+        pca_ss_rotation(ang[i], R + 9 * i);
+    }
+    return 0;
+}
+
+int pca_kitti_integrate_s(pca_ctx *ctx, pca_kitti_integrate_args *a, pca_kitti_step_state *s, int flags)
+{
+    if (!ctx) return -1;
+    if (!a || !s) { ctx->err = "kitti_integrate_s: no argument block"; return -1; }
+    if (!a->obs || !a->track || !a->T_new_prev || a->slot != s->tail) { ctx->err = "kitti_integrate_s: bad arguments"; return -1; }
+    const bool owes = s->tail > s->head && pca_host_track_len(a->track) > 0;
+    if (pca_ss_note(s, owes ? a->T_new_prev : nullptr, flags)) { ctx->err = "kitti_integrate_s: bad state block (slots, or the owed chain is full)"; return -1; }
+    return pca_kitti_integrate_v(ctx, a);
+}
+
+int pca_kitti_generate_bev_s(pca_ctx *ctx, pca_kitti_generate_bev_args *a, pca_kitti_step_state *s)
+{
+    if (!ctx) return -1;
+    ctx->bin_valid = false;
+    if (!a || !s) { ctx->err = "kitti_generate_bev_s: no argument block"; return -1; }
+    s->hinted = 0; s->n_rows = 0;
+    double chain_T[16 * PCA_BEV_MAX_CHAIN];
+    int32_t chain_ends[PCA_BEV_MAX_CHAIN];
+    if (!a->prm || pca_host_step_state_view(s, a->track, const_cast<pca_bev_params *>(a->prm), chain_T, chain_ends)) {
+        ctx->err = "kitti_generate_bev_s: bad state block (split outside the track, or an owed transform beyond the window)";
+        return -1;
+    }
+    const int F = s->tail - s->head;
+    if (s->cull && F >= 4 && !(s->n_pending > 0 && s->write_back)) {
+        if (!s->then || !s->box || !s->moved) { ctx->err = "kitti_generate_bev_s: no frame tables for the view hint"; return -1; }
+        const int rc = pca_bev_view_hint(ctx, s->head, F, s->then + 12 * (size_t)s->head, s->box + 6 * (size_t)s->head,
+                                         (s->cone && s->n_nocone == 0) ? s->cone : nullptr, s->moved, a->prm);
+        if (rc < 0) { ctx->err = "kitti_generate_bev_s: bad view hint"; return -1; }
+        s->hinted = rc;
+    }
+    return pca_kitti_generate_bev(ctx, a->store, a->frame_off, s->head, s->split, s->tail, a->max_points, a->prm, chain_T,
+                                  chain_ends, s->n_pending, s->write_back, a->workspace, a->workspace_bytes, a->planes_f16,
+                                  a->host_planes, a->track, a->traj_rows, a->traj_start, &s->n_rows, a->stream);
+}
+
+}
diff --git a/pc-accumulation-lib_amd/csrc/pca_step_state.h b/pc-accumulation-lib_amd/csrc/pca_step_state.h
--- /dev/null
+++ b/pc-accumulation-lib_amd/csrc/pca_step_state.h
@@ -0,0 +1,105 @@
+#pragma once
+#include <math.h>
+#include <stdint.h>
+#include <string.h>
+
+#include "../../include/pca.h"
+
+static inline void pca_ss_moved_step(double moved[16], const double T[16])
+{
+    double M[12];
+    for (int i = 0; i < 3; ++i)
+        for (int j = 0; j < 4; ++j)
+            M[4 * i + j] = fma(T[4 * i + 3], moved[12 + j], fma(T[4 * i + 2], moved[8 + j], fma(T[4 * i + 1], moved[4 + j], T[4 * i] * moved[j])));
+    memcpy(moved, M, sizeof(M));
+    moved[12] = 0.0; moved[13] = 0.0; moved[14] = 0.0; moved[15] = 1.0;
+}
+
+static inline int pca_ss_owe(pca_kitti_step_state *s, const double T[16])
+{
+    if (s->pend_n < 0 || s->pend_n >= PCA_BEV_MAX_CHAIN) return -1;
+    memcpy(s->pend_T + 16 * s->pend_n, T, 16 * sizeof(double));
+    s->pend_ends[s->pend_n] = s->tail;
+    s->pend_n++;
+    return 0;
+}
+
+static inline void pca_ss_drop_cones(pca_kitti_step_state *s)
+{
+    for (int32_t k = s->head; k < s->tail; ++k) s->has_cone[k] = 0;
+    s->n_nocone = s->tail - s->head;
+}
+
+static inline void pca_ss_note_frame(pca_kitti_step_state *s, int has_cone)
+{
+    memcpy(s->then + 12 * (size_t)s->tail, s->moved, 12 * sizeof(double));
+    s->has_cone[s->tail] = has_cone ? 1 : 0;
+    if (!has_cone) s->n_nocone++;
+}
+
+static inline int pca_ss_note(pca_kitti_step_state *s, const double *T, int flags)
+{
+    if (!s || !s->moved || !s->then || !s->has_cone || !s->pend_T || !s->pend_ends) return -1;
+    if (s->head < 0 || s->tail < s->head || s->tail >= s->slots) return -1;
+    if (T) {
+        if (s->pend_n < 0 || s->pend_n >= PCA_BEV_MAX_CHAIN) return -1;
+        pca_ss_moved_step(s->moved, T);
+        pca_ss_owe(s, T);
+    }
+    if (flags & 2) pca_ss_drop_cones(s);
+    pca_ss_note_frame(s, flags & 1);
+    return 0;
+}
+
+static inline int pca_ss_chain(const pca_kitti_step_state *s, double *chain_T, int32_t *chain_ends, int32_t *write_back)
+{
+    if (s->pend_n < 0 || s->pend_n > PCA_BEV_MAX_CHAIN) return -1;
+    if (s->pend_n == 0) { *write_back = 1; return 0; }
+    if (s->pend_ends[s->pend_n - 1] > s->tail) return -1;
+    int n = 0;
+    for (int k = 0; k < s->pend_n; ++k)
+        if (s->pend_ends[k] > s->head) {
+            memcpy(chain_T + 16 * n, s->pend_T + 16 * k, 16 * sizeof(double));
+            chain_ends[n++] = s->pend_ends[k];
+        }
+    *write_back = (n > 0 && n >= s->chain_k) ? 1 : 0;
+    return n;
+}
+
+static inline double pca_ss_heading(int has_step, double dx, double dy)
+{
+    double ang = 0.5 * M_PI;
+    if (has_step) ang += atan2(dy, dx);
+    return M_PI - ang;
+}
+
+static inline void pca_ss_rotation(double ang, double R[9])
+{
+    const double c = cos(ang), sn = sin(ang);
+    R[0] = c; R[1] = -sn; R[2] = 0.0;
+    R[3] = sn; R[4] = c; R[5] = 0.0;
+    R[6] = 0.0; R[7] = 0.0; R[8] = 1.0;
+}
+
+static inline int pca_ss_last_step(const double *poses, int64_t F, int64_t split, double dxy[2])
+{
+    if (!poses || split < 0 || split >= F) return -1;
+    dxy[0] = dxy[1] = 0.0;
+    if (split < 2) return 0;
+    const double *o = poses + 4 * split, *a = o - 8, *b = o - 4;
+    dxy[0] = (b[0] - o[0]) - (a[0] - o[0]);
+    dxy[1] = (b[1] - o[1]) - (a[1] - o[1]);
+    return 1;
+}
+
+static inline int pca_ss_view_head(const double *poses, int64_t F, int64_t split, double view, const double *ang, pca_bev_params *prm)
+{
+    if (!poses || !prm || split < 0 || split >= F) return -1;
+    const double *o = poses + 4 * split;
+    double dxy[2] = {0.0, 0.0};
+    const int has_step = ang ? 0 : pca_ss_last_step(poses, F, split, dxy);
+    prm->origin[0] = o[0]; prm->origin[1] = o[1]; prm->origin[2] = o[2];
+    pca_ss_rotation(ang ? *ang : pca_ss_heading(has_step, dxy[0], dxy[1]), prm->R);
+    prm->dx = 0.0; prm->dy = 0.0; prm->view = view;
+    return 0;
+}
diff --git a/pc-accumulation-lib_amd/kitti360_sem_pc_accum.py b/pc-accumulation-lib_amd/kitti360_sem_pc_accum.py
--- a/pc-accumulation-lib_amd/kitti360_sem_pc_accum.py
+++ b/pc-accumulation-lib_amd/kitti360_sem_pc_accum.py
@@ -34,8 +34,10 @@
         self._cobs = None
         self._ga = None
         self._ga_traj = None
+        self._ss_dxy = None
         self._fast = os.environ.get('PCA_FAST_CALLS', '1') != '0'
         self._defer_k1 = self._fast and os.environ.get('PCA_FUSE_K1', '1') != '0'
+        self._step_state = self._fast and os.environ.get('PCA_STEP_STATE', '1') != '0'
         self._prev_sweep = None
         self._sweep_dev = None
         self.pose_provider = self._default_pose_provider()
@@ -202,14 +204,15 @@
                 pc = dev
         fast = self._obs_pointers(rgb, pc, sem_gt) if self._fast else None
         general = self._frame_tensors(rgb, pc, sem_gt) if fast is None else None
-        if len(self._track) > 0:
+        owe = fast is not None and self._step_state
+        if not owe and len(self._track) > 0:
             self.update_sem_pcs(T_new_prev)
         if fast is not None:
             obs, semseg, H, W, keep = fast
             if self._defer_k1 != getattr(self.store.ctx, 'k1_defer', False):
                 self.store.set_defer_k1(self._defer_k1)
             idx, path_length = self.store.append_kitti_obs(obs, self.P_velo_frame, H, W, self.semseg_filters, self.sample_mode,
-                                                           self._track, T_new_prev, self.horizon_dist, keep=keep)
+                                                           self._track, T_new_prev, self.horizon_dist, keep=keep, owe=owe)
             del keep
             if idx is None:
                 idx, path_length = self._track.step(T_new_prev, self.horizon_dist)
@@ -322,14 +325,35 @@
         n = st.n_frames
         present_idx = int(present_idx)
         split = present_idx if present_idx >= 0 else n + present_idx
-        lo = max(split - 2, 0)
-        near = track.poses_window(lo, split + 1)
-        origin = near[split - lo]
-        rot_mat = hl.rotation_matrix_3d(hl.heading_rot_ang(near[:split - lo] - origin))
         px = gen.pixel_size
-        prm = gen._raster_params(origin, rot_mat, 0., 0., 1. * gen.view_size, st.intensity_div255)
+        sb = st.step_state_for_raster() if self._step_state else None
+        mode = hl.heading_mode() if sb is not None else 1
+        if mode != 1:
+            prm = gen._raster_block(st.intensity_div255)
+            sb.prm_ready = mode
+            if mode == 2:
+                ang = 0.5 * np.pi
+                sb.head, sb.split = st.head, st.head + split
+                has_step = ctx.lib.pca_host_step_state_last_step(st._ss_addr, track._h)
+                if has_step < 0:
+                    raise IndexError('present_idx outside the pose track')
+                if has_step:
+                    dxy = self._ss_dxy
+                    if dxy is None or dxy[0] is not sb:
+                        dxy = self._ss_dxy = (sb, np.frombuffer(sb.dxy, dtype=np.float64))
+                    ang += np.arctan2(dxy[1][1], dxy[1][0])
+                sb.ang = np.pi - ang
+        else:
+            lo = max(split - 2, 0)
+            near = track.poses_window(lo, split + 1)
+            origin = near[split - lo]
+            rot_mat = hl.rotation_matrix_3d(hl.heading_rot_ang(near[:split - lo] - origin))
+            prm = gen._raster_params(origin, rot_mat, 0., 0., 1. * gen.view_size, st.intensity_div255)
+            if sb is not None:
+                sb.prm_ready = 1
         max_points = st.bev_workspace(px)
-        n_pend, pend_T, pend_ends, write_back = st.bev_pending(0, n)
+        if sb is None:
+            n_pend, pend_T, pend_ends, write_back = st.bev_pending(0, n)
         if out is None:
             out = torch.empty((21, px, px), dtype=torch.float16, device=st.device)
         else:
@@ -345,6 +369,7 @@
         if a is None:
             from pca_amd._lib import PcaKittiGenerateBevArgs
             a = self._ga = PcaKittiGenerateBevArgs()
+            self._ga_addr = C.addressof(a)
             self._ga_const = None
         pend_T, pend_ends = st._pend_T, st._pend_ends
         const = (id(cst), id(st.frame_off), id(prm), id(pend_T), id(pend_ends), id(st._ws), track._h)
@@ -355,18 +380,28 @@
             a.track = getattr(track._h, 'value', track._h)
             self._ga_const = const
             self._ga_keep = (cst, st.frame_off, prm, pend_T, pend_ends, st._ws)
-        a.slot_begin, a.slot_split, a.slot_end, a.max_points = st.head, st.head + split, st.head + n, max_points
-        a.n_pending, a.write_back = n_pend, write_back
+        a.max_points = max_points
         a.planes_f16, a.host_planes = out.data_ptr(), (None if host is None else host.data_ptr())
         a.traj_rows, a.traj_start = self._ga_traj_addr
         a.stream = ctx.stream_int() or None
-        a.hint_F = st.view_hint_into(a, 0, n)
-        ticket = ctx.lib.pca_kitti_generate_bev_v(ctx.h, C.addressof(a))
-        if ticket < 0:
-            ctx.check(ticket)
-        st.hints_taken += a.hinted
+        if sb is not None:
+            sb.head, sb.split, sb.tail = st.head, st.head + split, st.head + n
+            sb.n_nocone, sb.cull, sb.view = st._n_nocone, (1 if st.cull else 0), 1. * gen.view_size
+            ticket = ctx.lib.pca_kitti_generate_bev_s(ctx.h, self._ga_addr, st._ss_addr)
+            if ticket < 0:
+                ctx.check(ticket)
+            hinted, n_rows, write_back = sb.hinted, sb.n_rows, sb.write_back
+        else:
+            a.slot_begin, a.slot_split, a.slot_end = st.head, st.head + split, st.head + n
+            a.n_pending, a.write_back = n_pend, write_back
+            a.hint_F = st.view_hint_into(a, 0, n)
+            ticket = ctx.lib.pca_kitti_generate_bev_v(ctx.h, self._ga_addr)
+            if ticket < 0:
+                ctx.check(ticket)
+            hinted, n_rows = a.hinted, a.n_rows
+        st.hints_taken += hinted
         st.bev_done(write_back)
-        rows = tb[0][:a.n_rows].copy()
+        rows = tb[0][:n_rows].copy()
         empty = np.zeros((0, 3))
         ego_p = rows[:start[split - 1]].copy() if split >= 2 else empty
         ego_f = rows[start[split]:].copy() if n - split >= 2 else empty
diff --git a/pc-accumulation-lib_amd/pca_amd/_lib.py b/pc-accumulation-lib_amd/pca_amd/_lib.py
--- a/pc-accumulation-lib_amd/pca_amd/_lib.py
+++ b/pc-accumulation-lib_amd/pca_amd/_lib.py
@@ -25,7 +25,7 @@
            'pca_host_track_append', 'pca_host_track_push_segment', 'pca_host_track_incr', 'pca_host_track_evict_beyond',
            'pca_host_track_step', 'pca_host_track_trigger', 'pca_host_stage_h2d', 'pca_host_d2h_async', 'pca_host_d2h_wait',
            'pca_deflate_workspace_bytes', 'pca_deflate_chunks', 'pca_deflate_chunks_dyn', 'pca_host_crc32_combine', 'pca_host_gzip_assemble',
-           'pca_kitti_integrate', 'pca_kitti_generate_bev', 'pca_k1_defer', 'pca_k1_flush', 'pca_host_camera_cone', 'pca_host_view_hull', 'pca_bev_bin_range', 'pca_bev_view_hint', 'pca_kitti_integrate_v', 'pca_kitti_generate_bev_v', 'pca_f32_box_decode', 'pca_debug_bev_level1', 'pca_debug_icp_layout',
+           'pca_kitti_integrate', 'pca_kitti_generate_bev', 'pca_k1_defer', 'pca_k1_flush', 'pca_host_camera_cone', 'pca_host_view_hull', 'pca_bev_bin_range', 'pca_bev_view_hint', 'pca_kitti_integrate_v', 'pca_kitti_generate_bev_v', 'pca_kitti_integrate_s', 'pca_kitti_generate_bev_s', 'pca_host_step_state_note', 'pca_host_step_state_view', 'pca_host_step_state_last_step', 'pca_host_heading_probe', 'pca_f32_box_decode', 'pca_debug_bev_level1', 'pca_debug_icp_layout',
            'pca_profile_enable', 'pca_profile_read')
 
 KERNEL_IDS = ('kitti_project_sample_filter', 'nusc_sample_filter_transform', 'nusc_project_cams', 'retransform',
@@ -55,6 +55,14 @@
                 ('pad1', C.c_int32), ('stream', C.c_void_p), ('hint_slot0', C.c_int32), ('hint_F', C.c_int32),
                 ('hint_then', C.c_void_p), ('hint_box', C.c_void_p), ('hint_cone', C.c_void_p), ('hint_now', C.c_void_p),
                 ('hinted', C.c_int32), ('pad2', C.c_int32)]
+
+
+class PcaKittiStepState(C.Structure):
+    _fields_ = [('moved', C.c_void_p), ('then', C.c_void_p), ('has_cone', C.c_void_p), ('box', C.c_void_p), ('pend_T', C.c_void_p),
+                ('pend_ends', C.c_void_p), ('cone', C.c_void_p), ('slots', C.c_int32), ('chain_k', C.c_int32), ('cull', C.c_int32),
+                ('prm_ready', C.c_int32), ('head', C.c_int32), ('tail', C.c_int32), ('split', C.c_int32), ('pend_n', C.c_int32),
+                ('n_nocone', C.c_int64), ('view', C.c_double), ('ang', C.c_double), ('dxy', C.c_double * 2), ('hinted', C.c_int32), ('n_rows', C.c_int32),
+                ('write_back', C.c_int32), ('n_pending', C.c_int32)]
 
 
 class PcaKittiObs(C.Structure):
@@ -248,6 +256,12 @@
     lib.pca_debug_icp_layout.argtypes = [i32, i32, C.POINTER(C.c_int64)]
     lib.pca_kitti_integrate_v.argtypes = [vp, vp]
     lib.pca_kitti_generate_bev_v.argtypes = [vp, vp]
+    lib.pca_kitti_integrate_s.argtypes = [vp, vp, vp, i32]
+    lib.pca_kitti_generate_bev_s.argtypes = [vp, vp, vp]
+    lib.pca_host_step_state_note.argtypes = [vp, vp, i32]
+    lib.pca_host_step_state_view.argtypes = [vp, vp, vp, vp, vp]
+    lib.pca_host_step_state_last_step.argtypes = [vp, vp]
+    lib.pca_host_heading_probe.argtypes = [vp, i64, i32, vp, vp]
     lib.pca_k1_defer.argtypes = [vp, i32]
     lib.pca_k1_flush.argtypes = [vp]
     lib.pca_profile_enable.argtypes = [vp, i32]
diff --git a/pc-accumulation-lib_amd/pca_amd/device_store.py b/pc-accumulation-lib_amd/pca_amd/device_store.py
--- a/pc-accumulation-lib_amd/pca_amd/device_store.py
+++ b/pc-accumulation-lib_amd/pca_amd/device_store.py
@@ -45,6 +45,10 @@
         self._pend_T = (C.c_double * (16 * self.CHAIN_MAX))()
         self._pend_T_np = np.frombuffer(self._pend_T, dtype=np.float64)
         self._pend_ends = (C.c_int * self.CHAIN_MAX)()
+        self._ss = None
+        self._ss_const = None
+        self._ss_last = None
+        self._ss_raw_ok = False
 
     def _alloc(self, cap):
         d = self.device
@@ -88,20 +92,28 @@
             M[3] = (0., 0., 0., 1.)
             self._moved = M
 
+    def _note_camera(self, cone_key):
+        if self._cone is not None and self._cone[0] == cone_key:
+            return False
+        other = self._cone is not None
+        out = np.empty(15)
+        Pm = np.frombuffer(cone_key[0], dtype=np.float64)
+        self.ctx.lib.pca_host_camera_cone(Pm.ctypes.data, int(cone_key[1]), int(cone_key[2]), out.ctypes.data)
+        self._cone = (cone_key, out, out.ctypes.data)
+        return other
+
     def _note_frame(self, slot, cone_key):
         self._then[slot] = self._moved[:3].reshape(12)
         if cone_key is not None:
-            if self._cone is None or self._cone[0] != cone_key:
-                if self._cone is not None:
-                    self._has_cone[self.head:self.tail] = False
-                    self._n_nocone = self.tail - self.head
-                out = np.empty(15)
-                Pm = np.frombuffer(cone_key[0], dtype=np.float64)
-                self.ctx.lib.pca_host_camera_cone(Pm.ctypes.data, int(cone_key[1]), int(cone_key[2]), out.ctypes.data)
-                self._cone = (cone_key, out, out.ctypes.data)
+            if self._note_camera(cone_key):
+                self._has_cone[self.head:self.tail] = False
+                self._n_nocone = self.tail - self.head
             self._has_cone[slot] = True
         else:
             self._n_nocone += 1
+        self._box_tick()
+
+    def _box_tick(self):
         self._since_box += 1
         self._poll_boxes()
         if self._since_box >= self.BOX_EVERY and self._box_copy is None:
@@ -150,6 +162,47 @@
     def _count_hint(self, r):
         self.hints_taken += 1 if r > 0 else 0
         return r
+
+    def _step_block(self):
+        b = self._ss
+        if b is None:
+            b = self._ss = _lib.PcaKittiStepState()
+            b.pend_T, b.pend_ends = C.addressof(self._pend_T), C.addressof(self._pend_ends)
+            b.chain_k = self.CHAIN_K
+            self._ss_addr = C.addressof(b)
+        cone = self._cone
+        const = (id(self._moved), id(self._then), id(self._has_cone), id(self._box), id(cone))
+        if const != self._ss_const:
+            if self._moved.dtype != np.float64 or not self._moved.flags.c_contiguous or self._moved.shape != (4, 4):
+                self._moved = np.ascontiguousarray(self._moved, dtype=np.float64).reshape(4, 4)
+                const = (id(self._moved), ) + const[1:]
+            b.moved, b.then, b.has_cone, b.box = self._moved.ctypes.data, self._then_addr, self._has_cone.ctypes.data, self._box_addr
+            b.cone = None if cone is None else cone[2]
+            b.slots = self._then.shape[0]
+            self._ss_const = const
+            self._ss_keep = (self._moved, self._then, self._has_cone, self._box, cone)
+        return b
+
+    def _chain_in_step(self):
+        p = self._pending
+        return self._ss_raw_ok and len(p) == self._ss.pend_n and (not p or p[-1] is self._ss_last)
+
+    def _chain_resync(self):
+        p = self._pending
+        for k, (T, e) in enumerate(p):
+            self._pend_T_np[16 * k:16 * k + 16] = T
+            self._pend_ends[k] = int(e)
+        self._ss.pend_n = len(p)
+        self._ss_last = p[-1] if p else None
+        self._ss_raw_ok = True
+
+    def step_state_for_raster(self):
+        if self._ss is None:
+            return None
+        p = self._pending
+        if not self._chain_in_step() or (p and p[-1][1] > self.tail):
+            return None
+        return self._step_block()
 
     def c_store(self):
         if self._cstore is None:
@@ -284,9 +337,15 @@
         self._ub += [int(f['pts'].shape[0]) for f in frames]
         self._ub_sum += n_in
 
-    def append_kitti_obs(self, obs, P, H, W, filters, sample_mode='nearest', track=None, T_new_prev=None, horizon=0., keep=None):
+    def append_kitti_obs(self, obs, P, H, W, filters, sample_mode='nearest', track=None, T_new_prev=None, horizon=0., keep=None,
+                         owe=False):
         lib, ctx = self.ctx.lib, self.ctx
         n = int(obs.n)
+        th = getattr(track, '_h', None)
+        native = owe and th is not None and self.tail + 1 <= self.max_frames and self.ub_tail + n <= self.capacity \
+            and len(self._pending) < self.CHAIN_MAX
+        if owe and not native and len(track) > 0:
+            self.retransform(np.asarray(T_new_prev, dtype=np.float64), defer=True)
         self.reserve(n, 1)
         src = self._k1_src
         if src is not None and src[0] is P and src[1] is filters and P.tobytes() == src[2] and tuple(filters or ()) == src[3]:
@@ -299,12 +358,12 @@
             self._k1_cache = (key, _lib.f64_array(P, 12), _lib.class_mask(filters))
         Pc, fmask = self._k1_cache[1], self._k1_cache[2]
         st = self.c_store()
-        th = getattr(track, '_h', None)
         a = self._ia
         if a is None:
             a = self._ia = _lib.PcaKittiIntegrateArgs()
             self._ia_T = np.zeros(16)
             self._ia_T_addr = self._ia_T.ctypes.data
+            self._ia_addr = C.addressof(a)
             self._ia_const = None
         const = (id(obs), id(Pc), int(H), int(W), id(st), id(self.frame_off), sample_mode, th, float(horizon))
         if const != self._ia_const:
@@ -320,9 +379,30 @@
         else:
             a.T_new_prev = None
         a.stream = ctx.stream_int() or None
-        ctx.check(lib.pca_kitti_integrate_v(ctx.h, C.addressof(a)))
-        self._k1_noted = (keep, ) if getattr(ctx, 'k1_defer', False) else None
-        self._note_frame(self.tail, (key[0], int(H), int(W)) if obs.sem_gt is None else None)
+        if native:
+            T16 = self._ia_T.copy()
+            flags = 0
+            if obs.sem_gt is None:
+                flags = 3 if self._note_camera((key[0], int(H), int(W))) else 1
+            b = self._step_block()
+            if not self._chain_in_step():
+                self._chain_resync()
+            owed = b.pend_n
+            b.head, b.tail, b.n_nocone = self.head, self.tail, self._n_nocone
+            if lib.pca_kitti_integrate_s(ctx.h, self._ia_addr, self._ss_addr, flags) != 0:
+                self._ss_raw_ok = False
+                ctx.check(-1)
+            if b.pend_n != owed:
+                self._ss_last = (T16, self.tail)
+                self._pending.append(self._ss_last)
+            if flags != 1:
+                self._n_nocone = int(b.n_nocone)
+            self._k1_noted = (keep, ) if getattr(ctx, 'k1_defer', False) else None
+            self._box_tick()
+        else:
+            ctx.check(lib.pca_kitti_integrate_v(ctx.h, C.addressof(a)))
+            self._k1_noted = (keep, ) if getattr(ctx, 'k1_defer', False) else None
+            self._note_frame(self.tail, (key[0], int(H), int(W)) if obs.sem_gt is None else None)
         self.tail += 1
         self.ub_tail += n
         self._ub.append(n)
@@ -499,6 +579,7 @@
         for T, e in self._pending:
             if e > self.head:
                 self._pend_T_np[16 * n_pend:16 * n_pend + 16] = T
+                self._ss_raw_ok = False
                 self._pend_ends[n_pend] = int(e)
                 n_pend += 1
         if n_pend == 0:
@@ -508,6 +589,8 @@
     def bev_done(self, write_back):
         if self._pending and write_back:
             self._pending = []
+            if self._ss is not None:
+                self._ss.pend_n, self._ss_last, self._ss_raw_ok = 0, None, True
         self._k1_noted = None
 
     def _side_workspace(self, name, workspace_bytes, max_points, px):
diff --git a/pc-accumulation-lib_amd/pca_amd/host_logic.py b/pc-accumulation-lib_amd/pca_amd/host_logic.py
--- a/pc-accumulation-lib_amd/pca_amd/host_logic.py
+++ b/pc-accumulation-lib_amd/pca_amd/host_logic.py
@@ -202,6 +202,133 @@
         if c is None or c[0] != ptr or c[1] < n:
             c = self._win = (ptr, n, self._view(ptr, n, 4))
         return c[2][first:last, :3].copy()
+
+    def pose(self, idx):
+        return self._P[idx].copy()
+
+    def as_array(self):
+        return self._P.copy()
+
+    def apply_transform(self, T):
+        if self._H.shape[0] == 0:
+            return
+        H = np.matmul(T, self._H)
+        H[:, 3, 0] = 1.0
+        self._H = H
+
+    def append(self, pose):
+        h = np.ones((1, 4, 1))
+        h[0, :3, 0] = np.asarray(pose, dtype=np.float64).reshape(3)
+        self._H = np.concatenate([self._H, h])
+
+    def push_segment(self):
+        self._D = np.append(self._D, pose_dist(self._H[-1, :3, 0], self._H[-2, :3, 0]))
+        return np.sum(self._D)
+
+    def evict_beyond(self, horizon_dist, path_length):
+        if not path_length > horizon_dist:
+            return 0
+        incr = incremental_path_dists(self._D)
+        incr -= path_length - horizon_dist
+        k = int((incr > 0.).argmax())
+        self._H = self._H[k:]
+        self._D = self._D[k:]
+        return k
+
+    def incr(self):
+        return incremental_path_dists(self._D)
+
+    def step(self, T_new_prev, horizon_dist):
+        if len(self) > 0:
+            self.apply_transform(T_new_prev)
+        self.append([0., 0., 0.])
+        if len(self) < 2:
+            return 0, None
+        path_length = self.push_segment()
+        return self.evict_beyond(horizon_dist, path_length), path_length
+
+    def trigger(self, bev_horizon, previous_idx, min_step):
+        if len(self) < 2:
+            return None
+        d = self.incr()
+        if d[-1] < bev_horizon:
+            return None
+        present_idx = int(((d - bev_horizon) > 0).argmax())
+        if d[-1] - d[present_idx] < bev_horizon:
+            return None
+        if pose_dist(self.pose(previous_idx), self.pose(present_idx)) < min_step:
+            return None
+        return present_idx
+
+
+def _numpy_gemv_entry():
+    import ctypes as C
+    try:
+        from threadpoolctl import threadpool_info
+        paths = [p['filepath'] for p in threadpool_info() if p.get('user_api') == 'blas' and p.get('filepath')]
+    except Exception:
+        return None
+    for path in paths:
+        try:
+            blas = C.CDLL(path)
+        except OSError:
+            continue
+        for sym in ('scipy_cblas_dgemv64_', 'cblas_dgemv64_'):
+            fn = getattr(blas, sym, None)
+            if fn is not None:
+                return C.cast(fn, C.c_void_p).value, blas
+    return None
+
+
+class CPoseTrack:
+    _lib = None
+    _gemv = None
+    _blas = None
+
+    def __init__(self):
+        import ctypes as C
+        self._C = C
+        h = C.c_void_p()
+        if self._lib.pca_host_track_create(C.byref(h), self._gemv) != 0:
+            raise RuntimeError('pca_host_track_create failed')
+        self._h = h
+        self._pl = C.c_double(0.0)
+        self._win = None
+
+    def __del__(self):
+        try:
+            self._lib.pca_host_track_destroy(self._h)
+        except Exception:
+            pass
+
+    def __len__(self):
+        return self._lib.pca_host_track_len(self._h)
+
+    def _view(self, ptr, n, width):
+        if n == 0:
+            return np.zeros((0, width)) if width > 1 else np.zeros(0)
+        a = np.ctypeslib.as_array((self._C.c_double * (n * width)).from_address(ptr))
+        return a.reshape(n, width) if width > 1 else a
+
+    def as_array(self):
+        n = len(self)
+        return self._view(self._lib.pca_host_track_poses(self._h), n, 4)[:, :3].copy()
+
+    def poses_window(self, first, last):
+        n = len(self)
+        ptr = self._lib.pca_host_track_poses(self._h)
+        c = self._win
+        if c is None or c[0] != ptr or c[1] < n:
+            c = self._win = (ptr, n, self._view(ptr, n, 4))
+        return c[2][first:last, :3].copy()
+
+    def poses_view(self):
+        n = len(self)
+        ptr = self._lib.pca_host_track_poses(self._h)
+        c = self._win
+        if c is None or c[0] != ptr or c[1] < n:
+            c = self._win = (ptr, n, self._view(ptr, n, 4))
+        return c[2]
 
     def pose(self, idx):
         n = len(self)
@@ -348,6 +475,34 @@
     return np.pi - ang
 
 
+_HEADING_MODE = []
+
+
+def heading_mode():
+    if not _HEADING_MODE:
+        import os
+        mode = 1
+        lib = _c_library()
+        if os.environ.get('PCA_HOST_HEADING', 'c') != 'numpy' and lib is not None and hasattr(lib, 'pca_host_heading_probe'):
+            rng = np.random.default_rng(20261020)
+            n = 4096
+            d = rng.normal(size=(n, 2)) * rng.choice([1e-6, 1e-2, 1., 1e2], size=(n, 1))
+            d[:8] = [[0., 0.], [-0., 0.], [0., -0.], [-0., -0.], [1., 0.], [-1., 0.], [0., 1.], [0., -1.]]
+            d[8:16, 1] = 0.
+            d[16:24, 0] = 0.
+            want_ang = np.array([heading_rot_ang([[0., 0.], [x, y]]) for x, y in d], dtype=np.float64)
+            want = np.stack([rotation_matrix_3d(a).reshape(9).astype(np.float64) for a in want_ang])
+            for given in (0, 1):
+                ang, got = want_ang.copy(), np.empty((n, 9))
+                if lib.pca_host_heading_probe(d.ctypes.data, n, given, ang.ctypes.data, got.ctypes.data) == 0 \
+                        and np.array_equal(ang.view(np.uint64), want_ang.view(np.uint64)) \
+                        and np.array_equal(got.view(np.uint64), want.view(np.uint64)):
+                    mode = 2 if given else 0
+                    break
+        _HEADING_MODE.append(mode)
+    return _HEADING_MODE[0]
+
+
 def pos2grid_inplace(mat, view, px):
     mat[:, 0:2] = np.floor(mat[:, 0:2] / view * px + 0.5 * px)
     return mat
```

New measurement: 1582 Mpoints/s, median of 2. No clear change (-0.0%).
